# cvg/LightGlue

Hardware: AMD Instinct MI355X
Metric: image-pairs/s at N=M=1024, 9 layers; match-index parity vs ref (higher is better)
Workload: dtype f16; 1 GPU; SuperPoint-dim 256-d descriptors, N=M=1024, 9 layers, pruning/early-stop OFF, batch=32 pairs per GPU, seeded random weights (recipe A), precision=f16x3 (split-f16 operands, 3 MFMAs per product, for every contraction incl. q k^T and P V; fp32 accumulate / residual / softmax); pairs_per_gpu=32, keypoints=1024, keypoints1=1024, descriptor_dim=256, parallelism=pair-sharded dp1, batches_in_flight=1

## Files before the change

### include/lightglue_amd.h

```cpp
#ifndef LIGHTGLUE_AMD_H
#define LIGHTGLUE_AMD_H

#include <stdint.h>

#ifdef __cplusplus
extern "C" {
#endif

enum {
    LG_PREC_F32 = 0,
    LG_PREC_BF16 = 1,
    LG_PREC_F16 = 2,
    LG_PREC_F16X3 = 4
};

#define LG_OK 0
#define LG_ERR_INVALID 1
#define LG_ERR_HIP 2
#define LG_ERR_STATE 3
#define LG_ERR_RANGE 4
#define LG_ERR_DEVICE 5
#define LG_ERR_INDEX 6

#define LG_WIRE_WIDTH(n0, n1) (3LL * (n0) + 3LL * (n1) + 2)
#define LG_MAX_KEYPOINTS 8192
#define LG_MAX_ROWS 2097152
#define LG_MAX_SIM_ELEMS 2147483647LL

typedef struct lg_config {
    int32_t input_dim;
    int32_t descriptor_dim;
    int32_t n_layers;
    int32_t num_heads;
    int32_t add_scale_ori;
    double depth_confidence;
    double width_confidence;
    double filter_threshold;
    int32_t pruning_min_kpts;
    int32_t precision;
    int32_t attn_precision;
} lg_config;

typedef struct lg_engine lg_engine;

#define LG_FLAG_NO_PRUNING 1u
#define LG_FLAG_EXT 2u
#define LG_FLAG_CHECK_FINITE 4u

#define LG_FLAG_INDEXED 8u

typedef struct lg_forward_io {
    int32_t batch, n0, n1;
    uint32_t flags;
    const float *kpts0, *kpts1;
    const float *desc0, *desc1;
    const float *size0, *size1;
    const float *scales0, *oris0, *scales1, *oris1;
    int32_t *matches0, *matches1;
    float *scores0, *scores1;
    int32_t *stop;
    int32_t *prune0, *prune1;
    int32_t *matches;
    float *match_scores;
    int32_t *n_matches;
    const int32_t *num0, *num1;
    float *log_assignment;
    int64_t *matches0_i64, *matches1_i64;
    int64_t *matches_i64;
    int64_t *stop_i64;
    int64_t *prune0_i64, *prune1_i64;
    float *prune0_f32, *prune1_f32;
    int32_t *wire; int64_t wire_stride;
    int32_t *status;
    const int32_t *index0, *index1;
    int32_t images0, images1;
} lg_forward_io;

const char* lg_last_error(void);
const char* lg_version(void);

int lg_engine_create(const lg_config* cfg, lg_engine** out);
void lg_engine_destroy(lg_engine* e);

int lg_engine_set_weight(lg_engine* e, const char* name, const float* host_data, const int64_t* shape, int32_t ndim);
int lg_engine_finalize_weights(lg_engine* e);

int lg_engine_reserve(lg_engine* e, int32_t max_batch, int32_t max_n0, int32_t max_n1);

int lg_engine_forward(lg_engine* e, const lg_forward_io* io, void* hip_stream);

typedef struct lg_unpack_io {
    const int32_t *wire; int64_t wire_stride; int32_t rows;
    int32_t n0, n1, with_prune, pairs_out;
    const int32_t *order;
    int64_t *matches0, *matches1, *stop;
    float *scores0, *scores1;
    int64_t *prune0_i64, *prune1_i64; float *prune0_f32, *prune1_f32;
    int64_t *matches; float *match_scores;
    int32_t *info;
} lg_unpack_io;
int lg_unpack_wire(const lg_unpack_io* io, void* hip_stream);

int lg_engine_set_option(lg_engine* e, const char* key, int32_t value);

int lg_debug_mfma_sustained(double* tflops, double* mhz, void* hip_stream);
int lg_engine_debug_stop_after(lg_engine* e, int32_t step);
int lg_engine_debug_read(lg_engine* e, const char* name, void* host_dst, int64_t max_bytes, int64_t* nbytes_out);
int lg_engine_debug_caps(lg_engine* e, int32_t* cap0, int32_t* cap1);

int32_t lg_profile_num_classes(void);
const char* lg_profile_class_name(int32_t cls);
int lg_engine_profile_enable(lg_engine* e, int32_t on);
int lg_engine_profile_read(lg_engine* e, double* ms, int64_t* count, int32_t n_classes);

int lg_sp_sample_descriptors(const float* desc_map, int32_t batch, int32_t channels, int32_t h, int32_t w,
                             const float* keypoints, const int32_t* num, int32_t n, int32_t cell,
                             int32_t normalize_dense, float* workspace, float* out, void* hip_stream);

int lg_sp_pack_conv_weight(const float* src, int32_t cout, int32_t cin, int32_t k, float* dst, void* hip_stream);
int64_t lg_sp_encode_workspace_bytes(int32_t batch, int32_t h, int32_t w);
int lg_sp_encode(const float* image, int32_t batch, int32_t h, int32_t w, const float* const* params, void* workspace,
                 int64_t workspace_bytes, float* scores, float* desc_map, void* hip_stream);
int lg_sp_pack_conv_weight_split(const float* src, int32_t cout, int32_t cin, int32_t k, void* dst, void* hip_stream);
int lg_sp_encode_split(const float* image, int32_t batch, int32_t h, int32_t w, const float* const* params, void* workspace,
                       int64_t workspace_bytes, float* scores, float* desc_map, void* hip_stream);

int64_t lg_sp_detect_workspace_bytes(int32_t batch, int32_t h, int32_t w, int32_t max_candidates);
int lg_sp_detect(const float* scores, int32_t batch, int32_t h, int32_t w, int32_t nms_radius, int32_t remove_borders,
                 float detection_threshold, int32_t max_keypoints, int32_t capacity, int32_t max_candidates,
                 void* workspace, int64_t workspace_bytes, float* keypoints, float* kp_scores, int32_t* counts,
                 int32_t* totals, void* hip_stream);

int64_t lg_aliked_packed_bytes(int32_t n_pos);
int lg_aliked_pack_weights(int32_t n_pos, const float* const* tensors, int32_t n_tensors, void* packed, int64_t packed_bytes, void* hip_stream);
int64_t lg_aliked_levels_bytes(int32_t batch, int32_t h, int32_t w);
int64_t lg_aliked_workspace_bytes(int32_t batch, int32_t h, int32_t w, int32_t n_pos);
int lg_aliked_encode(const float* image, int32_t batch, int32_t channels, int32_t h, int32_t w, int32_t n_pos, const void* packed, void* levels,
                     void* workspace, int64_t workspace_bytes, float* scores, void* hip_stream);
int64_t lg_aliked_detect_workspace_bytes(int32_t batch, int32_t h, int32_t w, int32_t capacity);
int lg_aliked_detect(const float* scores, int32_t batch, int32_t h, int32_t w, const float* image_size, int32_t nms_radius, float scores_th,
                     int32_t top_k, int32_t n_limit, int32_t capacity, void* workspace, int64_t workspace_bytes, float* keypoints,
                     float* kp_scores, float* kp_norm, int32_t* counts, void* hip_stream);
int64_t lg_aliked_describe_workspace_bytes(int32_t rows, int32_t n_pos);
int lg_aliked_describe(const void* levels, int32_t batch, int32_t h, int32_t w, int32_t n_pos, const void* packed, const float* kp_norm,
                       const int32_t* counts, int32_t n, void* workspace, int64_t workspace_bytes, float* descriptors, void* hip_stream);

#define LG_PREPROCESS_MAX_TAPS 33
#define LG_PREPROCESS_MAX_SIDE 8388608
#define LG_RESIZE_EDGE (-1)
enum { LG_SIDE_LONG = 0, LG_SIDE_SHORT = 1, LG_SIDE_VERT = 2, LG_SIDE_HORZ = 3 };
enum { LG_DTYPE_F32 = 0, LG_DTYPE_U8 = 1 };
typedef struct lg_resize_plan {
    int32_t h_in, w_in, h_out, w_out;
    int32_t ks_y, ks_x;
    int32_t align_corners;
    int32_t identity;
    double sigma_y, sigma_x;
    double scale_x, scale_y;
} lg_resize_plan;
int lg_preprocess_plan(int32_t h, int32_t w, int32_t resize_h, int32_t resize_w, int32_t side, int32_t antialias, int32_t align_corners,
                       lg_resize_plan* plan);
int lg_preprocess_resize(const void* src, int32_t dtype, int32_t batch, int32_t channels, int32_t h, int32_t w, int64_t stride_b,
                         int64_t stride_c, int64_t stride_y, int64_t stride_x, const lg_resize_plan* plan, float* dst, void* hip_stream);

#ifdef __cplusplus
}
#endif
#endif
```

### lightglue_amd/_cabi.py

```python
from __future__ import annotations

import ctypes as C
import os
from pathlib import Path

_LIB_PATH = Path(os.environ.get("LIGHTGLUE_AMD_LIB") or Path(__file__).resolve().parent / "liblightglue_amd.so")

LG_PREC = {"fp32": 0, "bf16": 1, "fp16": 2, "f16x3": 4}
LG_OK, LG_ERR_INVALID, LG_ERR_HIP, LG_ERR_STATE, LG_ERR_RANGE, LG_ERR_DEVICE, LG_ERR_INDEX = 0, 1, 2, 3, 4, 5, 6
LG_FLAG_NO_PRUNING, LG_FLAG_EXT, LG_FLAG_CHECK_FINITE, LG_FLAG_INDEXED = 1, 2, 4, 8
LG_MAX_KEYPOINTS, LG_MAX_ROWS, LG_MAX_SIM_ELEMS = 8192, 2 ** 21, 2 ** 31 - 1

EXPORTED_SYMBOLS = (
    "lg_last_error", "lg_version", "lg_engine_create", "lg_engine_destroy", "lg_engine_set_weight",
    "lg_engine_finalize_weights", "lg_engine_reserve", "lg_engine_forward", "lg_unpack_wire", "lg_engine_set_option",
    "lg_engine_debug_stop_after", "lg_engine_debug_read", "lg_engine_debug_caps",
    "lg_profile_num_classes", "lg_profile_class_name", "lg_engine_profile_enable", "lg_engine_profile_read",
    "lg_sp_sample_descriptors", "lg_sp_detect_workspace_bytes", "lg_sp_detect",
    "lg_sp_pack_conv_weight", "lg_sp_encode_workspace_bytes", "lg_sp_encode", "lg_sp_pack_conv_weight_split", "lg_sp_encode_split", "lg_debug_mfma_sustained",
    "lg_aliked_packed_bytes", "lg_aliked_pack_weights", "lg_aliked_levels_bytes", "lg_aliked_workspace_bytes", "lg_aliked_encode",
    "lg_aliked_detect_workspace_bytes", "lg_aliked_detect", "lg_aliked_describe_workspace_bytes", "lg_aliked_describe",
    "lg_preprocess_plan", "lg_preprocess_resize",
)


class LgConfig(C.Structure):
    _fields_ = [
        ("input_dim", C.c_int32), ("descriptor_dim", C.c_int32), ("n_layers", C.c_int32), ("num_heads", C.c_int32),
        ("add_scale_ori", C.c_int32),
        ("depth_confidence", C.c_double), ("width_confidence", C.c_double), ("filter_threshold", C.c_double),
        ("pruning_min_kpts", C.c_int32), ("precision", C.c_int32), ("attn_precision", C.c_int32),
    ]


_fp = C.c_void_p


class LgForwardIO(C.Structure):
    _fields_ = [
        ("batch", C.c_int32), ("n0", C.c_int32), ("n1", C.c_int32), ("flags", C.c_uint32),
        ("kpts0", _fp), ("kpts1", _fp), ("desc0", _fp), ("desc1", _fp), ("size0", _fp), ("size1", _fp),
        ("scales0", _fp), ("oris0", _fp), ("scales1", _fp), ("oris1", _fp),
        ("matches0", _fp), ("matches1", _fp), ("scores0", _fp), ("scores1", _fp), ("stop", _fp),
        ("prune0", _fp), ("prune1", _fp), ("matches", _fp), ("match_scores", _fp), ("n_matches", _fp),
        ("num0", _fp), ("num1", _fp), ("log_assignment", _fp),
        ("matches0_i64", _fp), ("matches1_i64", _fp), ("matches_i64", _fp), ("stop_i64", _fp),
        ("prune0_i64", _fp), ("prune1_i64", _fp), ("prune0_f32", _fp), ("prune1_f32", _fp),
        ("wire", _fp), ("wire_stride", C.c_int64), ("status", _fp),
        ("index0", _fp), ("index1", _fp), ("images0", C.c_int32), ("images1", C.c_int32),
    ]


class LgUnpackIO(C.Structure):
    _fields_ = [
        ("wire", _fp), ("wire_stride", C.c_int64), ("rows", C.c_int32),
        ("n0", C.c_int32), ("n1", C.c_int32), ("with_prune", C.c_int32), ("pairs_out", C.c_int32),
        ("order", _fp),
        ("matches0", _fp), ("matches1", _fp), ("stop", _fp),
        ("scores0", _fp), ("scores1", _fp),
        ("prune0_i64", _fp), ("prune1_i64", _fp), ("prune0_f32", _fp), ("prune1_f32", _fp),
        ("matches", _fp), ("match_scores", _fp),
        ("info", _fp),
    ]


LG_PREPROCESS_MAX_TAPS, LG_PREPROCESS_MAX_SIDE, LG_RESIZE_EDGE = 33, 2 ** 23, -1
LG_SIDE = {"long": 0, "short": 1, "vert": 2, "horz": 3}
LG_DTYPE_F32, LG_DTYPE_U8 = 0, 1


class LgResizePlan(C.Structure):
    _fields_ = [
        ("h_in", C.c_int32), ("w_in", C.c_int32), ("h_out", C.c_int32), ("w_out", C.c_int32),
        ("ks_y", C.c_int32), ("ks_x", C.c_int32), ("align_corners", C.c_int32), ("identity", C.c_int32),
        ("sigma_y", C.c_double), ("sigma_x", C.c_double), ("scale_x", C.c_double), ("scale_y", C.c_double),
    ]


def wire_width(n0: int, n1: int) -> int:
    return 3 * n0 + 3 * n1 + 2


class LightGlueAmdError(RuntimeError):
    pass


_lib = None


def library_path() -> Path:
    return _LIB_PATH


def load() -> C.CDLL:
    global _lib
    if _lib is not None:
        return _lib
    if not _LIB_PATH.exists():
        raise LightGlueAmdError(
            f"{_LIB_PATH} is missing: build it with `python -c 'import __graft_entry__ as g; g.build()'` "
            f"or `make -C {_LIB_PATH.parent / 'csrc'}`; lightglue_amd has no CPU / PyTorch fallback.")
    lib = C.CDLL(os.fspath(_LIB_PATH))
    lib.lg_last_error.restype = C.c_char_p
    lib.lg_version.restype = C.c_char_p
    lib.lg_engine_create.argtypes = [C.POINTER(LgConfig), C.POINTER(C.c_void_p)]
    lib.lg_engine_destroy.argtypes = [C.c_void_p]
    lib.lg_engine_destroy.restype = None
    lib.lg_engine_set_weight.argtypes = [C.c_void_p, C.c_char_p, C.c_void_p, C.POINTER(C.c_int64), C.c_int32]
    lib.lg_engine_finalize_weights.argtypes = [C.c_void_p]
    lib.lg_engine_reserve.argtypes = [C.c_void_p, C.c_int32, C.c_int32, C.c_int32]
    lib.lg_engine_forward.argtypes = [C.c_void_p, C.POINTER(LgForwardIO), C.c_void_p]
    lib.lg_unpack_wire.argtypes = [C.POINTER(LgUnpackIO), C.c_void_p]
    lib.lg_engine_set_option.argtypes = [C.c_void_p, C.c_char_p, C.c_int32]
    lib.lg_engine_debug_stop_after.argtypes = [C.c_void_p, C.c_int32]
    lib.lg_engine_debug_read.argtypes = [C.c_void_p, C.c_char_p, C.c_void_p, C.c_int64, C.POINTER(C.c_int64)]
    lib.lg_engine_debug_caps.argtypes = [C.c_void_p, C.POINTER(C.c_int32), C.POINTER(C.c_int32)]
    lib.lg_profile_num_classes.restype = C.c_int32
    lib.lg_profile_class_name.restype = C.c_char_p
    lib.lg_profile_class_name.argtypes = [C.c_int32]
    lib.lg_engine_profile_enable.argtypes = [C.c_void_p, C.c_int32]
    lib.lg_engine_profile_read.argtypes = [C.c_void_p, C.POINTER(C.c_double), C.POINTER(C.c_int64), C.c_int32]
    lib.lg_sp_sample_descriptors.argtypes = [C.c_void_p, C.c_int32, C.c_int32, C.c_int32, C.c_int32, C.c_void_p, C.c_void_p,
                                             C.c_int32, C.c_int32, C.c_int32, C.c_void_p, C.c_void_p, C.c_void_p]
    lib.lg_sp_detect_workspace_bytes.argtypes = [C.c_int32] * 4
    lib.lg_sp_detect_workspace_bytes.restype = C.c_int64
    lib.lg_sp_detect.argtypes = [C.c_void_p] + [C.c_int32] * 5 + [C.c_float] + [C.c_int32] * 3 + [C.c_void_p, C.c_int64] + [C.c_void_p] * 5
    lib.lg_sp_pack_conv_weight.argtypes = [C.c_void_p, C.c_int32, C.c_int32, C.c_int32, C.c_void_p, C.c_void_p]
    lib.lg_sp_encode_workspace_bytes.argtypes = [C.c_int32] * 3
    lib.lg_sp_encode_workspace_bytes.restype = C.c_int64
    lib.lg_sp_encode.argtypes = [C.c_void_p, C.c_int32, C.c_int32, C.c_int32, C.POINTER(C.c_void_p), C.c_void_p, C.c_int64, C.c_void_p, C.c_void_p, C.c_void_p]
    lib.lg_sp_pack_conv_weight_split.argtypes = lib.lg_sp_pack_conv_weight.argtypes
    lib.lg_sp_encode_split.argtypes = lib.lg_sp_encode.argtypes
    lib.lg_aliked_packed_bytes.argtypes = [C.c_int32]
    lib.lg_aliked_packed_bytes.restype = C.c_int64
    lib.lg_aliked_pack_weights.argtypes = [C.c_int32, C.POINTER(C.c_void_p), C.c_int32, C.c_void_p, C.c_int64, C.c_void_p]
    lib.lg_aliked_levels_bytes.argtypes = [C.c_int32] * 3
    lib.lg_aliked_levels_bytes.restype = C.c_int64
    lib.lg_aliked_workspace_bytes.argtypes = [C.c_int32] * 4
    lib.lg_aliked_workspace_bytes.restype = C.c_int64
    lib.lg_aliked_encode.argtypes = [C.c_void_p] + [C.c_int32] * 5 + [C.c_void_p] * 3 + [C.c_int64, C.c_void_p, C.c_void_p]
    lib.lg_aliked_detect_workspace_bytes.argtypes = [C.c_int32] * 4
    lib.lg_aliked_detect_workspace_bytes.restype = C.c_int64
    lib.lg_aliked_detect.argtypes = ([C.c_void_p] + [C.c_int32] * 3 + [C.c_void_p, C.c_int32, C.c_float] + [C.c_int32] * 3
                                     + [C.c_void_p, C.c_int64] + [C.c_void_p] * 5)
    lib.lg_aliked_describe_workspace_bytes.argtypes = [C.c_int32] * 2
    lib.lg_aliked_describe_workspace_bytes.restype = C.c_int64
    lib.lg_aliked_describe.argtypes = [C.c_void_p] + [C.c_int32] * 4 + [C.c_void_p] * 3 + [C.c_int32, C.c_void_p, C.c_int64, C.c_void_p, C.c_void_p]
    lib.lg_preprocess_plan.argtypes = [C.c_int32] * 7 + [C.POINTER(LgResizePlan)]
    lib.lg_preprocess_resize.argtypes = [C.c_void_p] + [C.c_int32] * 5 + [C.c_int64] * 4 + [C.POINTER(LgResizePlan), C.c_void_p, C.c_void_p]
    lib.lg_debug_mfma_sustained.argtypes = [C.POINTER(C.c_double), C.POINTER(C.c_double), C.c_void_p]
    _lib = lib
    return lib


def check(rc: int) -> None:
    if rc == LG_OK:
        return
    msg = load().lg_last_error().decode()
    if rc == LG_ERR_INVALID:
        raise AssertionError(msg)
    raise LightGlueAmdError(f"lightglue_amd error {rc}: {msg}")
```

### lightglue_amd/csrc/lg_attention.hip

```cpp
#include "lg_kernels.h"

namespace lg {

constexpr int ABK = 64, ATHREADS = 256;

#ifdef LG_ATTN_TIMING
struct PhaseClock { long long tacc[7] = {0, 0, 0, 0, 0, 0, 0}, tprev = clock64(); };
#define ATT_TICK(pc, slot) do { const long long _n = clock64(); (pc).tacc[slot] += _n - (pc).tprev; (pc).tprev = _n; } while (0)
#else
struct PhaseClock {};
#define ATT_TICK(pc, slot) do { } while (0)
#endif
#ifdef LG_ATTN_WALL
struct WallClock { long long wall0 = wall_clock64(), cyc0 = clock64(); };
#else
struct WallClock {};
#endif
template <int NW> __device__ __forceinline__ long long* dbg_words(const AttnArgs& a) {
    return a.dbg && (threadIdx.x & 63) == 0 ? a.dbg + ((long long)blockIdx.x * NW + (threadIdx.x >> 6)) * 8 : nullptr;
}
template <int NW> __device__ __forceinline__ void dump_timing(const AttnArgs& a, const PhaseClock& pc, int ntiles) {
#ifdef LG_ATTN_TIMING
    if (long long* d = dbg_words<NW>(a)) {
        for (int i = 0; i < 6; ++i) d[i] = pc.tacc[i];
        d[6] = ntiles; d[7] = 1;
    }
#endif
}
template <int NW> __device__ __forceinline__ void dump_wall(const AttnArgs& a, const WallClock& wc, int ntiles) {
#ifdef LG_ATTN_WALL
    if (long long* d = dbg_words<NW>(a)) {
        d[0] = wc.wall0; d[1] = wall_clock64(); d[2] = clock64() - wc.cyc0; d[3] = __builtin_amdgcn_s_getreg((31 << 11) | 4); d[4] = __builtin_amdgcn_s_getreg((31 << 11) | 20); d[6] = ntiles; d[7] = 1;
    }
#endif
}

static int attention_tiles(const RowSpace& rs, int rows) {
    return rows <= 128 ? rs.B * (rs.cap0 + rs.cap1) / rows : rs.B * ((rs.cap0 + rows - 1) / rows + (rs.cap1 + rows - 1) / rows);
}
struct AttnWg { int head; TileLoc t; int qlen, kvseg, kvlen; long long kvbase; };
template <int ABM> __device__ __forceinline__ bool attn_workgroup(const AttnArgs& a, AttnWg& w) {
    const int ntile = gridDim.x >> 2;
    const int v = xcd_remap(blockIdx.x, gridDim.x);
    w.head = v / ntile;
    TileLoc& t = w.t;
    if constexpr (ABM <= 128) {
        t = locate_tile(a.rs, v - w.head * ntile, ABM);
    } else {
        const int t0 = (a.rs.cap0 + ABM - 1) / ABM, t1 = (a.rs.cap1 + ABM - 1) / ABM, idx = v - w.head * ntile;
        t.pair = idx / (t0 + t1);
        const int rem = idx - t.pair * (t0 + t1);
        t.image = rem >= t0 ? 1 : 0;
        t.r0 = (rem - t.image * t0) * ABM;
        t.seg = 2 * t.pair + t.image;
        t.grow0 = seg_row_base(a.rs, t.seg) + t.r0;
    }
    w.qlen = a.rs.len[t.seg];
    if (t.r0 >= w.qlen) return false;
    if (a.rs.active && !a.rs.active[t.pair]) return false;
    w.kvseg = a.cross ? (t.seg ^ 1) : t.seg;
    w.kvlen = a.rs.len[w.kvseg];
    w.kvbase = seg_row_base(a.rs, w.kvseg);
    return true;
}
template <int ABM, int NT> __device__ __forceinline__ void zero_ctx_tile(float* ctx, const AttnWg& w, int tid) {
    for (int i = tid; i < ABM * 16; i += NT) {
        const int row = i >> 4, c4 = i & 15;
        if (w.t.r0 + row < w.qlen) *reinterpret_cast<f32x4*>(ctx + (w.t.grow0 + row) * 256LL + w.head * 64 + c4 * 4) = f32x4{0.f, 0.f, 0.f, 0.f};
    }
}
template <int EPC> __device__ __forceinline__ constexpr int key_of(int kt, int g, int r) {
    return EPC == 8 ? 32 * (kt >> 1) + 8 * g + 4 * (kt & 1) + r : 16 * kt + 4 * g + r;
}
template <int EPC, int QT> __device__ __forceinline__ void mask_dead_keys(f32x4 (&s)[4][QT], const int& g, const int& kv0, const int& kvlen) {
    if (kv0 + ABK > kvlen) {
#pragma unroll
        for (int qt = 0; qt < QT; ++qt)
#pragma unroll
            for (int kt = 0; kt < 4; ++kt)
#pragma unroll
                for (int r = 0; r < 4; ++r)
                    if (kv0 + key_of<EPC>(kt, g, 0) + r >= kvlen) s[kt][qt][r] = -INFINITY;
    }
}
template <int QT> __device__ __forceinline__ float row_max16(const f32x4 (&s)[4][QT], int qt) {
    const float t0 = vmax3(s[0][qt][0], s[0][qt][1], s[0][qt][2]), t1 = vmax3(s[0][qt][3], s[1][qt][0], s[1][qt][1]);
    const float t2 = vmax3(s[1][qt][2], s[1][qt][3], s[2][qt][0]), t3 = vmax3(s[2][qt][1], s[2][qt][2], s[2][qt][3]);
    const float t4 = vmax3(s[3][qt][0], s[3][qt][1], s[3][qt][2]);
    const float mx = vmax2(vmax3(t0, t1, t2), vmax3(t3, t4, s[3][qt][3]));
    return xor32_max(xor16_max(mx));
}
template <bool SUB_M, int QT> __device__ __forceinline__ void exp_sum(f32x4 (&s)[4][QT], const float (&m_run)[QT], float (&l_run)[QT]) {
#pragma unroll
    for (int qt = 0; qt < QT; ++qt) {
        const float nm = m_run[qt];
        auto ex = [&](float x) { if constexpr (SUB_M) return __builtin_amdgcn_exp2f(x - nm); else return __builtin_amdgcn_exp2f(x); };
        float rs0 = 0.f, rs1 = 0.f;
#pragma unroll
        for (int kt = 0; kt < 4; ++kt) {
            const float p0 = ex(s[kt][qt][0]), p1 = ex(s[kt][qt][1]);
            const float p2 = ex(s[kt][qt][2]), p3 = ex(s[kt][qt][3]);
            s[kt][qt][0] = p0; s[kt][qt][1] = p1; s[kt][qt][2] = p2; s[kt][qt][3] = p3;
            rs0 += p0 + p2; rs1 += p1 + p3;
        }
        l_run[qt] += rs0 + rs1;
    }
}
template <int QT> __device__ __forceinline__ void start_rebased(f32x4 (&o)[4][QT], float (&m_run)[QT], float (&l_run)[QT]) {
#pragma unroll
    for (int qt = 0; qt < QT; ++qt) {
        m_run[qt] = 0.f; l_run[qt] = 0.f;
#pragma unroll
        for (int i = 0; i < 4; ++i) o[i][qt] = f32x4{0.f, 0.f, 0.f, 0.f};
    }
}
template <int QT> __device__ __forceinline__ void softmax_rebase(f32x4 (&s)[4][QT], f32x4 (&o)[4][QT], float (&m_run)[QT], float (&l_run)[QT],
                                                                 bool first, int g, int kv0, int kvlen) {
    mask_dead_keys<8>(s, g, kv0, kvlen);
    float dmax[QT];
    bool grew = first;
#pragma unroll
    for (int qt = 0; qt < QT; ++qt) {
        dmax[qt] = row_max16(s, qt);
        grew = grew || (dmax[qt] > 8.f);
    }
    if (__any(grew)) {
#pragma unroll
        for (int qt = 0; qt < QT; ++qt) {
            const float shift = first ? dmax[qt] : (dmax[qt] > 8.f ? dmax[qt] : 0.f);
            const float alpha = first ? 0.f : __builtin_amdgcn_exp2f(-shift);
            l_run[qt] *= alpha;
#pragma unroll
            for (int dt = 0; dt < 4; ++dt) o[dt][qt] *= alpha;
            m_run[qt] += shift;
#pragma unroll
            for (int kt = 0; kt < 4; ++kt) s[kt][qt] -= shift;
        }
    }
}
template <int QT> __device__ __forceinline__ void store_ctx(float* ctx, const TileLoc& t, int head, int qlen, int wave, int lr, int g,
                                                            const f32x4 (&o)[4][QT], const float (&l_run)[QT]) {
#pragma unroll
    for (int qt = 0; qt < QT; ++qt) {
        float l = l_run[qt];
        l = xor32_sum(xor16_sum(l));
        const float inv = 1.f / l;
        const int qrow = t.r0 + wave * (16 * QT) + qt * 16 + lr;
        if (qrow < qlen) {
            float* dst = ctx + (t.grow0 + wave * (16 * QT) + qt * 16 + lr) * 256LL + head * 64 + g * 4;
#pragma unroll
            for (int dt = 0; dt < 4; ++dt) *reinterpret_cast<f32x4*>(dst + dt * 16) = o[dt][qt] * inv;
        }
    }
}
template <class Tag> __device__ __forceinline__ u32x4 mask_tail(u32x4 v, int nvalid) {
    constexpr int EPC = Tag::EPC;
    if (nvalid >= EPC) return v;
    if (nvalid <= 0) return u32x4{0u, 0u, 0u, 0u};
    if constexpr (EPC == 4) {
#pragma unroll
        for (int i = 0; i < 4; ++i) if (i >= nvalid) v[i] = 0u;
    } else {
#pragma unroll
        for (int i = 0; i < 4; ++i) {
            if (2 * i >= nvalid) v[i] = 0u;
            else if (2 * i + 1 >= nvalid) v[i] &= 0xFFFFu;
        }
    }
    return v;
}
__device__ __forceinline__ int k_swz128(int row) { return ((row >> 1) & 1) | (((row >> 3) & 3) << 1); }
template <int ROWB> __device__ __forceinline__ int k_off(int row, int slot16) {
    if constexpr (ROWB == 128) return row * 128 + ((slot16 ^ k_swz128(row)) << 4);
    else return lds_off<ROWB>(row, slot16);
}
template <int PPW, class T> __device__ __forceinline__ void dma_lanes(int wave, int lane, const T* Vt, int head, long long R, long long kvbase,
                                                                      int (&koff)[PPW], const T* (&vrow)[PPW]) {
    const int prow = lane >> 3, pslot = lane & 7;
    int voff[PPW];
#pragma unroll
    for (int i = 0; i < PPW; ++i) {
        const int row = (PPW * wave + i) * 8 + prow;
        koff[i] = row * 64 + ((pslot ^ k_swz128(row)) << 3);
        voff[i] = (pslot ^ lds_swz128(row)) << 3;
    }
#pragma unroll
    for (int i = 0; i < PPW; ++i) vrow[i] = Vt + ((long long)head * 64 + (PPW * wave + i) * 8 + prow) * R + kvbase + voff[i];
}
__device__ __forceinline__ void frag_bases(int lr, int g, int vt, int (&kfo)[2], int (&vfo)[2]) {
#pragma unroll
    for (int c = 0; c < 2; ++c) {
        kfo[c] = k_off<128>(key_of<8>(0, lr >> 2, lr & 3), c * 4 + g);
        vfo[c] = vt + lds_off<128>(lr, 4 * c + g);
    }
}
__device__ __forceinline__ void set_priority_by_progress(int tile, int ntiles) {
    if ((tile & 3) == 0) {
        const int q = (tile * 4) / ntiles;
        if (q == 0) __builtin_amdgcn_s_setprio(3); else if (q == 1) __builtin_amdgcn_s_setprio(2); else if (q == 2) __builtin_amdgcn_s_setprio(1); else __builtin_amdgcn_s_setprio(0);
    }
}
__device__ __forceinline__ void publish_tile() {
    wait_vmcnt0();
    asm volatile("" ::: "memory");
    __syncthreads();
}

template <class Tag, int QT>
__global__ __launch_bounds__(ATHREADS) void attn_kernel(AttnArgs a) {
    constexpr int ABM = 64 * QT;
    typedef typename Tag::elem T;
    constexpr int EPC = Tag::EPC;
    constexpr int ROWB = 64 * (int)sizeof(T);
    constexpr int SLOTS = ROWB / 16;
    constexpr int NC = 64 / (4 * EPC);
    constexpr int NCT = 64 * SLOTS / ATHREADS;
    extern __shared__ __attribute__((aligned(16))) char smem[];
    char* bK = smem;
    char* bV = smem + 64 * ROWB;

    AttnWg w;
    if (!attn_workgroup<ABM>(a, w)) return;
    const int head = w.head, kvlen = w.kvlen;
    const long long kvbase = w.kvbase;
    const int tid = threadIdx.x, lane = tid & 63, wave = tid >> 6, lr = lane & 15, g = lane >> 4;
    const long long R = a.R;
    const T* Q = static_cast<const T*>(a.q);
    const T* Kp = static_cast<const T*>(a.cross ? a.q : a.k);
    const T* Vt = static_cast<const T*>(a.vt);

    if (kvlen == 0) { zero_ctx_tile<ABM, ATHREADS>(a.ctx, w, tid); return; }

    u32x4 qf[QT][NC];
#pragma unroll
    for (int qt = 0; qt < QT; ++qt) {
        const long long grow = min((long long)w.t.grow0 + wave * (16 * QT) + qt * 16 + lr, R - 1);
#pragma unroll
        for (int c = 0; c < NC; ++c)
            qf[qt][c] = *reinterpret_cast<const u32x4*>(Q + ((long long)head * R + grow) * 64 + c * 4 * EPC + g * EPC);
    }

    f32x4 o[4][QT];
    float m_run[QT], l_run[QT];
#pragma unroll
    for (int qt = 0; qt < QT; ++qt) {
        m_run[qt] = -INFINITY; l_run[qt] = 0.f;
#pragma unroll
        for (int i = 0; i < 4; ++i) o[i][qt] = f32x4{0.f, 0.f, 0.f, 0.f};
    }

    u32x4 rk[NCT], rv[NCT];
    auto load_tile = [&](int kv0) {
#pragma unroll
        for (int i = 0; i < NCT; ++i) {
            const int c = tid + ATHREADS * i, row = c / SLOTS, slot = c % SLOTS;
            rk[i] = *reinterpret_cast<const u32x4*>(Kp + ((long long)head * R + kvbase + kv0 + row) * 64 + slot * EPC);
            rv[i] = *reinterpret_cast<const u32x4*>(Vt + ((long long)head * 64 + row) * R + kvbase + kv0 + slot * EPC);
        }
    };
    auto store_tile = [&](int kv0) {
        if (kv0 + ABK <= kvlen) {
#pragma unroll
            for (int i = 0; i < NCT; ++i) {
                const int c = tid + ATHREADS * i, row = c / SLOTS, slot = c % SLOTS;
                *reinterpret_cast<u32x4*>(bK + k_off<ROWB>(row, slot)) = rk[i];
                *reinterpret_cast<u32x4*>(bV + lds_off<ROWB>(row, slot)) = rv[i];
            }
        } else {
#pragma unroll
            for (int i = 0; i < NCT; ++i) {
                const int c = tid + ATHREADS * i, row = c / SLOTS, slot = c % SLOTS;
                const u32x4 kz = (kv0 + row < kvlen) ? rk[i] : u32x4{0u, 0u, 0u, 0u};
                *reinterpret_cast<u32x4*>(bK + k_off<ROWB>(row, slot)) = kz;
                *reinterpret_cast<u32x4*>(bV + lds_off<ROWB>(row, slot)) = mask_tail<Tag>(rv[i], kvlen - (kv0 + slot * EPC));
            }
        }
    };

    const int ntiles = (kvlen + ABK - 1) / ABK;
    PhaseClock pc;
    auto qk = [&](f32x4 (&s)[4][QT]) {
#pragma unroll
        for (int kt = 0; kt < 4; ++kt)
#pragma unroll
            for (int qt = 0; qt < QT; ++qt) s[kt][qt] = f32x4{0.f, 0.f, 0.f, 0.f};
#pragma unroll
        for (int c = 0; c < NC; ++c) {
#pragma unroll
            for (int kt = 0; kt < 4; ++kt) {
                const u32x4 kf = *reinterpret_cast<const u32x4*>(bK + k_off<ROWB>(key_of<EPC>(kt, lr >> 2, lr & 3), c * 4 + g));
#pragma unroll
                for (int qt = 0; qt < QT; ++qt) mma_chunk<Tag>(s[kt][qt], kf, qf[qt][c]);
            }
        }
    };
    auto smax_rescale = [&](f32x4 (&s)[4][QT], int kv0) {
        mask_dead_keys<EPC>(s, g, kv0, kvlen);
        float m_new[QT];
        bool grew = false;
#pragma unroll
        for (int qt = 0; qt < QT; ++qt) {
            m_new[qt] = vmax2(m_run[qt], row_max16(s, qt));
            grew = grew || (m_new[qt] > m_run[qt] + 8.f);
        }
        if (__any(grew)) {
#pragma unroll
            for (int qt = 0; qt < QT; ++qt) {
                const float m_upd = m_new[qt] > m_run[qt] + 8.f ? m_new[qt] : m_run[qt];
                const float alpha = __builtin_amdgcn_exp2f(m_run[qt] - m_upd);
                l_run[qt] *= alpha;
#pragma unroll
                for (int dt = 0; dt < 4; ++dt) o[dt][qt] *= alpha;
                m_run[qt] = m_upd;
            }
        }
    };
    auto pv = [&](f32x4 (&s)[4][QT]) {
        if constexpr (EPC == 8) {
#pragma unroll
            for (int tp = 0; tp < 2; ++tp) {
                u32x4 pp[QT];
#pragma unroll
                for (int qt = 0; qt < QT; ++qt) pp[qt] = pack8<Tag>(s[2 * tp][qt], s[2 * tp + 1][qt]);
#pragma unroll
                for (int dt = 0; dt < 4; ++dt) {
                    const u32x4 vf = *reinterpret_cast<const u32x4*>(bV + lds_off<ROWB>(dt * 16 + lr, 4 * tp + g));
#pragma unroll
                    for (int qt = 0; qt < QT; ++qt) mma_chunk<Tag>(o[dt][qt], vf, pp[qt]);
                }
            }
        } else {
#pragma unroll
            for (int kt = 0; kt < 4; ++kt) {
#pragma unroll
                for (int dt = 0; dt < 4; ++dt) {
                    const u32x4 vf = *reinterpret_cast<const u32x4*>(bV + lds_off<ROWB>(dt * 16 + lr, 4 * kt + g));
#pragma unroll
                    for (int qt = 0; qt < QT; ++qt) mma_chunk<Tag>(o[dt][qt], vf, __builtin_bit_cast(u32x4, s[kt][qt]));
                }
            }
        }
    };

    load_tile(0);
    f32x4 s[4][QT];
    for (int tile = 0; tile < ntiles; ++tile) {
        const int kv0 = tile * ABK;
        __syncthreads();
        ATT_TICK(pc, 0);
        store_tile(kv0);
        __syncthreads();
        ATT_TICK(pc, 1);
        load_tile(tile + 1 < ntiles ? kv0 + ABK : kv0);
        __builtin_amdgcn_sched_barrier(0);
        qk(s);
        ATT_TICK(pc, 2);
        smax_rescale(s, kv0);
        exp_sum<true>(s, m_run, l_run);
        ATT_TICK(pc, 4);
        pv(s);
        ATT_TICK(pc, 5);
    }
    dump_timing<4>(a, pc, ntiles);
    store_ctx(a.ctx, w.t, head, w.qlen, wave, lr, g, o, l_run);
}

template <class Tag>
__global__ __launch_bounds__(ATHREADS, 4) void attn_dma_kernel(AttnArgs a) {
    constexpr int QT = 2, ABM = 128, ROWB = 128, TILEB = 64 * ROWB, BUFB = 2 * TILEB;
    typedef typename Tag::elem T;
    extern __shared__ __attribute__((aligned(16))) char smem[];

    AttnWg w;
    if (!attn_workgroup<ABM>(a, w)) return;
    const int head = w.head, kvlen = w.kvlen;
    const long long kvbase = w.kvbase;
    const int tid = threadIdx.x, lane = tid & 63, wave = __builtin_amdgcn_readfirstlane(tid >> 6), lr = lane & 15, g = lane >> 4;
    const long long R = a.R;
    const T* Q = static_cast<const T*>(a.q);
    const T* Kp = static_cast<const T*>(a.cross ? a.q : a.k);
    const T* Vt = static_cast<const T*>(a.vt);

    if (kvlen == 0) { zero_ctx_tile<ABM, ATHREADS>(a.ctx, w, tid); return; }

    int koff[2];
    const T* vrow[2];
    dma_lanes<2>(wave, lane, Vt, head, R, kvbase, koff, vrow);
    const T* kseg = Kp + ((long long)head * R + kvbase) * 64;
    auto dma_tile = [&](int buf, int kv0) {
        char* bK = smem + buf * BUFB; char* bV = bK + TILEB;
#pragma unroll
        for (int i = 0; i < 2; ++i) {
            lds_dma16(kseg + (long long)kv0 * 64 + koff[i], bK + (2 * wave + i) * 1024);
            lds_dma16(vrow[i] + kv0, bV + (2 * wave + i) * 1024);
        }
    };
    dma_tile(0, 0);

    int kfo[2], vfo[2];
    frag_bases(lr, g, TILEB, kfo, vfo);
    u32x4 qf[QT][2];
#pragma unroll
    for (int qt = 0; qt < QT; ++qt) {
        const long long grow = (long long)w.t.grow0 + wave * 32 + qt * 16 + lr;
#pragma unroll
        for (int c = 0; c < 2; ++c) qf[qt][c] = *reinterpret_cast<const u32x4*>(Q + ((long long)head * R + grow) * 64 + c * 32 + g * 8);
    }
    f32x4 o[4][QT];
    float m_run[QT], l_run[QT];
    start_rebased(o, m_run, l_run);

    const int ntiles = (kvlen + ABK - 1) / ABK;
    PhaseClock pc;
    WallClock wc;
    for (int tile = 0; tile < ntiles; ++tile) {
        const int kv0 = tile * ABK;
        const char* bK = smem + (tile & 1) * BUFB; const char* bV = bK + TILEB;
        set_priority_by_progress(tile, ntiles);
        publish_tile();
        ATT_TICK(pc, 0);
        if (kv0 + ABK > kvlen) {
#pragma unroll
            for (int i = 0; i < 2; ++i) {
                const int c = tid + ATHREADS * i, row = c >> 3, slot = c & 7;
                u32x4* p = reinterpret_cast<u32x4*>(const_cast<char*>(bV) + lds_off<ROWB>(row, slot));
                *p = mask_tail<Tag>(*p, kvlen - (kv0 + slot * 8));
            }
            __syncthreads();
        }
        dma_tile((tile + 1) & 1, tile + 1 < ntiles ? kv0 + ABK : kv0);
        __builtin_amdgcn_sched_barrier(0);
        ATT_TICK(pc, 1);

        f32x4 s[4][QT];
#pragma unroll
        for (int kt = 0; kt < 4; ++kt)
#pragma unroll
            for (int qt = 0; qt < QT; ++qt) s[kt][qt] = f32x4{-m_run[qt], -m_run[qt], -m_run[qt], -m_run[qt]};
#pragma unroll
        for (int c = 0; c < 2; ++c) {
#pragma unroll
            for (int kt = 0; kt < 4; ++kt) {
                const u32x4 kf = *reinterpret_cast<const u32x4*>(bK + kfo[c] + key_of<8>(kt, 0, 0) * ROWB);
#pragma unroll
                for (int qt = 0; qt < QT; ++qt) mma_chunk<Tag>(s[kt][qt], kf, qf[qt][c]);
            }
        }
        ATT_TICK(pc, 2);
        softmax_rebase(s, o, m_run, l_run, tile == 0, g, kv0, kvlen);
        ATT_TICK(pc, 3);
        exp_sum<false>(s, m_run, l_run);
        ATT_TICK(pc, 4);
#pragma unroll
        for (int tp = 0; tp < 2; ++tp) {
            u32x4 pp[QT];
#pragma unroll
            for (int qt = 0; qt < QT; ++qt) pp[qt] = pack8<Tag>(s[2 * tp][qt], s[2 * tp + 1][qt]);
#pragma unroll
            for (int dt = 0; dt < 4; ++dt) {
                const u32x4 vf = *reinterpret_cast<const u32x4*>(bK + vfo[tp] + dt * 16 * ROWB);
#pragma unroll
                for (int qt = 0; qt < QT; ++qt) mma_chunk<Tag>(o[dt][qt], vf, pp[qt]);
            }
        }
        ATT_TICK(pc, 5);
    }
    asm volatile("s_waitcnt vmcnt(0)" ::: "memory");
    dump_timing<4>(a, pc, ntiles);
    dump_wall<4>(a, wc, ntiles);
    store_ctx(a.ctx, w.t, head, w.qlen, wave, lr, g, o, l_run);
}

template <int QT> __device__ __forceinline__ void mma_pair(f32x4 (&acc)[4][QT], int first, const u32x4 (&a)[2], const u32x4 (&b)[QT][2], int c) {
#pragma unroll
    for (int j = 0; j < 2; ++j)
#pragma unroll
        for (int qt = 0; qt < QT; ++qt) mma_chunk<TagF16>(acc[first + j][qt], a[j], b[qt][c]);
}
template <int QT, int NW>
__global__ __launch_bounds__(NW * 64, NW / 2) void attn_split_kernel(AttnArgs a) {
    typedef TagF16 Tag;
    typedef f16_t T;
    constexpr int NT = NW * 64, PPW = 8 / NW;
    constexpr int ABM = 16 * QT * NW, ROWB = 128, TILEB = 64 * ROWB, BUFB = 4 * TILEB;
    extern __shared__ __attribute__((aligned(16))) char smem[];

    AttnWg w;
    if (!attn_workgroup<ABM>(a, w)) return;
    const int head = w.head, kvlen = w.kvlen;
    const long long kvbase = w.kvbase;
    const int tid = threadIdx.x, lane = tid & 63, wave = __builtin_amdgcn_readfirstlane(tid >> 6), lr = lane & 15, g = lane >> 4;
    const long long R = a.R, PL = a.plane;
    const T* Q = static_cast<const T*>(a.q);
    const T* Kp = static_cast<const T*>(a.cross ? a.q : a.k);
    const T* Vt = static_cast<const T*>(a.vt);

    if (kvlen == 0) { zero_ctx_tile<ABM, NT>(a.ctx, w, tid); return; }

    int koff[PPW];
    const T* vrow[PPW];
    dma_lanes<PPW>(wave, lane, Vt, head, R, kvbase, koff, vrow);
    const T* kseg = Kp + ((long long)head * R + kvbase) * 64;
    auto dma_tile = [&](int buf, int kv0) {
        char* bK = smem + buf * BUFB;
#pragma unroll
        for (int i = 0; i < PPW; ++i) {
            const T* ks = kseg + (long long)kv0 * 64 + koff[i];
            const T* vs = vrow[i] + kv0;
            char* dst = bK + (PPW * wave + i) * 1024;
            lds_dma16(ks, dst); lds_dma16(ks + PL, dst + TILEB);
            lds_dma16(vs, dst + 2 * TILEB); lds_dma16(vs + PL, dst + 3 * TILEB);
        }
    };
    dma_tile(0, 0);

    int kfo[2], vfo[2];
    frag_bases(lr, g, 2 * TILEB, kfo, vfo);
    u32x4 qh[QT][2], ql[QT][2];
#pragma unroll
    for (int qt = 0; qt < QT; ++qt) {
        const long long grow = (long long)w.t.grow0 + wave * (16 * QT) + qt * 16 + lr;
#pragma unroll
        for (int c = 0; c < 2; ++c) {
            const T* src = Q + ((long long)head * R + grow) * 64 + c * 32 + g * 8;
            qh[qt][c] = *reinterpret_cast<const u32x4*>(src);
            ql[qt][c] = *reinterpret_cast<const u32x4*>(src + PL);
        }
    }
    f32x4 o[4][QT];
    float m_run[QT], l_run[QT];
    start_rebased(o, m_run, l_run);

    const int ntiles = (kvlen + ABK - 1) / ABK;
    PhaseClock pc;
    WallClock wc;
    for (int tile = 0; tile < ntiles; ++tile) {
        const int kv0 = tile * ABK;
        const char* bK = smem + (tile & 1) * BUFB;
        set_priority_by_progress(tile, ntiles);
        publish_tile();
        ATT_TICK(pc, 0);
        if (kv0 + ABK > kvlen) {
#pragma unroll
            for (int i = 0; i < 1024 / NT; ++i) {
                const int c = (tid + NT * i) & 511, plane = (tid + NT * i) >> 9, row = c >> 3, slot = c & 7;
                u32x4* p = reinterpret_cast<u32x4*>(const_cast<char*>(bK) + (2 + plane) * TILEB + lds_off<ROWB>(row, slot));
                *p = mask_tail<Tag>(*p, kvlen - (kv0 + slot * 8));
            }
            __syncthreads();
        }
        u32x4 fh[2][2], fl[2][2];
        auto load_k = [&](int grp, u32x4 (&h)[2], u32x4 (&l)[2]) {
            const int c = grp >> 1, kp = grp & 1;
#pragma unroll
            for (int j = 0; j < 2; ++j) {
                const char* src = bK + kfo[c] + key_of<8>(2 * kp + j, 0, 0) * ROWB;
                h[j] = *reinterpret_cast<const u32x4*>(src);
                l[j] = *reinterpret_cast<const u32x4*>(src + TILEB);
            }
        };
        auto load_v = [&](int grp, u32x4 (&h)[2], u32x4 (&l)[2]) {
            const int tp = grp >> 1, dp = grp & 1;
#pragma unroll
            for (int j = 0; j < 2; ++j) {
                const char* src = bK + vfo[tp] + (2 * dp + j) * 16 * ROWB;
                h[j] = *reinterpret_cast<const u32x4*>(src);
                l[j] = *reinterpret_cast<const u32x4*>(src + TILEB);
            }
        };
        load_k(0, fh[0], fl[0]);
        dma_tile((tile + 1) & 1, tile + 1 < ntiles ? kv0 + ABK : kv0);
        __builtin_amdgcn_sched_barrier(0);
        ATT_TICK(pc, 1);

        f32x4 s[4][QT];
#pragma unroll
        for (int kt = 0; kt < 4; ++kt)
#pragma unroll
            for (int qt = 0; qt < QT; ++qt) s[kt][qt] = f32x4{-m_run[qt], -m_run[qt], -m_run[qt], -m_run[qt]};
#pragma unroll
        for (int grp = 0; grp < 4; ++grp) {
            const int c = grp >> 1, kp = grp & 1;
            if (grp < 3) load_k(grp + 1, fh[(grp + 1) & 1], fl[(grp + 1) & 1]);
            else load_v(0, fh[0], fl[0]);
            __builtin_amdgcn_sched_barrier(0);
            const u32x4 (&kh)[2] = fh[grp & 1];
            const u32x4 (&kl)[2] = fl[grp & 1];
            mma_pair(s, 2 * kp, kh, ql, c);
            mma_pair(s, 2 * kp, kl, qh, c);
            mma_pair(s, 2 * kp, kh, qh, c);
            __builtin_amdgcn_sched_barrier(0);
        }
        ATT_TICK(pc, 2);
        softmax_rebase(s, o, m_run, l_run, tile == 0, g, kv0, kvlen);
        ATT_TICK(pc, 3);
        exp_sum<false>(s, m_run, l_run);
        ATT_TICK(pc, 4);
        u32x4 ph[QT][2], pl[QT][2];
#pragma unroll
        for (int tp = 0; tp < 2; ++tp)
#pragma unroll
            for (int qt = 0; qt < QT; ++qt) split8_f16<true>(s[2 * tp][qt], s[2 * tp + 1][qt], ph[qt][tp], pl[qt][tp]);
#pragma unroll
        for (int grp = 0; grp < 4; ++grp) {
            const int tp = grp >> 1, dp = grp & 1;
            if (grp < 3) load_v(grp + 1, fh[(grp + 1) & 1], fl[(grp + 1) & 1]);
            __builtin_amdgcn_sched_barrier(0);
            const u32x4 (&vh)[2] = fh[grp & 1];
            const u32x4 (&vl)[2] = fl[grp & 1];
            mma_pair(o, 2 * dp, vh, pl, tp);
            mma_pair(o, 2 * dp, vl, ph, tp);
            mma_pair(o, 2 * dp, vh, ph, tp);
            __builtin_amdgcn_sched_barrier(0);
        }
        ATT_TICK(pc, 5);
    }
    asm volatile("s_waitcnt vmcnt(0)" ::: "memory");
    dump_timing<NW>(a, pc, ntiles);
    dump_wall<NW>(a, wc, ntiles);
    store_ctx(a.ctx, w.t, head, w.qlen, wave, lr, g, o, l_run);
}

template <int QT, int NW> static hipError_t launch_attn_split(const AttnArgs& a, hipStream_t s) {
    if (a.plane <= 0) return hipErrorInvalidValue;
    constexpr int smem = 2 * 4 * 64 * 128;
    auto kern = attn_split_kernel<QT, NW>;
    hipError_t e = hipFuncSetAttribute(reinterpret_cast<const void*>(kern), hipFuncAttributeMaxDynamicSharedMemorySize, smem);
    if (e != hipSuccess) return e;
    hipLaunchKernelGGL(kern, dim3(attention_tiles(a.rs, 16 * QT * NW) * 4), dim3(NW * 64), smem, s, a);
    return hipGetLastError();
}

template <class Tag> static hipError_t launch_attn_dma(const AttnArgs& a, hipStream_t s) {
    hipLaunchKernelGGL((attn_dma_kernel<Tag>), dim3(attention_tiles(a.rs, 128) * 4), dim3(ATHREADS), 2 * 2 * 64 * 128, s, a);
    return hipGetLastError();
}

template <class Tag, int QT> static hipError_t launch_attn_t(const AttnArgs& a, hipStream_t s) {
    constexpr int smem = 2 * 64 * 64 * (int)sizeof(typename Tag::elem);
    hipLaunchKernelGGL((attn_kernel<Tag, QT>), dim3(attention_tiles(a.rs, 64 * QT) * 4), dim3(ATHREADS), smem, s, a);
    return hipGetLastError();
}

template <class Tag> static hipError_t launch_attn_16bit(const AttnArgs& a, hipStream_t s) {
    const int rpw = a.rows_per_wave;
    if (a.dma && rpw == 32) return launch_attn_dma<Tag>(a, s);
    return rpw == 64 ? launch_attn_t<Tag, 4>(a, s) : rpw == 16 ? launch_attn_t<Tag, 1>(a, s) : launch_attn_t<Tag, 2>(a, s);
}

hipError_t launch_attention(int attn_prec, const AttnArgs& a, hipStream_t s) {
    switch (attn_prec) {
        case PREC_F32: return launch_attn_t<TagF32, 2>(a, s);
        case PREC_BF16: return launch_attn_16bit<TagBF16>(a, s);
        case PREC_F16: return launch_attn_16bit<TagF16>(a, s);
        case PREC_F16X3: return a.rows_per_wave == 16 ? launch_attn_split<1, 4>(a, s) : launch_attn_split<1, 8>(a, s);
    }
    return hipErrorInvalidValue;
}

}
```

### lightglue_amd/csrc/lg_common.h

```cpp
#pragma once
#include <hip/hip_runtime.h>
#include <stdint.h>

#if defined(__HIP_DEVICE_COMPILE__) && !defined(__gfx950__)
#error "lightglue_amd kernels are gfx950 (MI355X, CDNA4) only: build with --offload-arch=gfx950"
#endif

namespace lg {

typedef __bf16 bf16_t;
typedef _Float16 f16_t;
typedef float f32x4 __attribute__((ext_vector_type(4)));
typedef float f32x2 __attribute__((ext_vector_type(2)));
typedef __bf16 bf16x8 __attribute__((ext_vector_type(8)));
typedef __bf16 bf16x4 __attribute__((ext_vector_type(4)));
typedef _Float16 f16x8 __attribute__((ext_vector_type(8)));
typedef _Float16 f16x4 __attribute__((ext_vector_type(4)));
typedef uint32_t u32x4 __attribute__((ext_vector_type(4)));
typedef uint32_t u32x2 __attribute__((ext_vector_type(2)));

enum : int { PREC_F32 = 0, PREC_BF16 = 1, PREC_F16 = 2, PREC_F16X3 = 4 };
__host__ __device__ constexpr bool prec_is_split(int prec) { return prec == PREC_F16X3; }

struct TagF32 { typedef float elem; static constexpr int EPC = 4; };
struct TagBF16 { typedef bf16_t elem; static constexpr int EPC = 8; };
struct TagF16 { typedef f16_t elem; static constexpr int EPC = 8; };

template <class Tag> __device__ __forceinline__ void mma_chunk(f32x4& acc, const u32x4& a, const u32x4& b);
template <> __device__ __forceinline__ void mma_chunk<TagBF16>(f32x4& acc, const u32x4& a, const u32x4& b) {
    acc = __builtin_amdgcn_mfma_f32_16x16x32_bf16(__builtin_bit_cast(bf16x8, a), __builtin_bit_cast(bf16x8, b), acc, 0, 0, 0);
}
template <> __device__ __forceinline__ void mma_chunk<TagF16>(f32x4& acc, const u32x4& a, const u32x4& b) {
    acc = __builtin_amdgcn_mfma_f32_16x16x32_f16(__builtin_bit_cast(f16x8, a), __builtin_bit_cast(f16x8, b), acc, 0, 0, 0);
}
template <> __device__ __forceinline__ void mma_chunk<TagF32>(f32x4& acc, const u32x4& a, const u32x4& b) {
    const f32x4 af = __builtin_bit_cast(f32x4, a), bf = __builtin_bit_cast(f32x4, b);
    acc = __builtin_amdgcn_mfma_f32_16x16x4f32(af[0], bf[0], acc, 0, 0, 0);
    acc = __builtin_amdgcn_mfma_f32_16x16x4f32(af[1], bf[1], acc, 0, 0, 0);
    acc = __builtin_amdgcn_mfma_f32_16x16x4f32(af[2], bf[2], acc, 0, 0, 0);
    acc = __builtin_amdgcn_mfma_f32_16x16x4f32(af[3], bf[3], acc, 0, 0, 0);
}

__device__ __forceinline__ uint32_t pack2_bf16(float a, float b) {
    typedef __bf16 bf16x2 __attribute__((ext_vector_type(2)));
    bf16x2 v = {(bf16_t)a, (bf16_t)b};
    return __builtin_bit_cast(uint32_t, v);
}
__device__ __forceinline__ uint32_t pack2_f16(float a, float b) {
    typedef _Float16 f16x2 __attribute__((ext_vector_type(2)));
    f16x2 v = {(f16_t)a, (f16_t)b};
    return __builtin_bit_cast(uint32_t, v);
}
template <class Tag> __device__ __forceinline__ uint32_t pack2(float a, float b);
template <> __device__ __forceinline__ uint32_t pack2<TagBF16>(float a, float b) { return pack2_bf16(a, b); }
template <> __device__ __forceinline__ uint32_t pack2<TagF16>(float a, float b) { return pack2_f16(a, b); }

template <class Tag> __device__ __forceinline__ u32x4 pack8(const f32x4& lo, const f32x4& hi) {
    u32x4 r;
    r[0] = pack2<Tag>(lo[0], lo[1]); r[1] = pack2<Tag>(lo[2], lo[3]);
    r[2] = pack2<Tag>(hi[0], hi[1]); r[3] = pack2<Tag>(hi[2], hi[3]);
    return r;
}
__device__ __forceinline__ void split2_f16(float a, float b, uint32_t& hi, uint32_t& lo) {
    hi = pack2_f16(a, b);
    float la, lb;
    asm("v_fma_mix_f32 %0, %1, -1.0, %2 op_sel_hi:[1,0,0]" : "=v"(la) : "v"(hi), "v"(a));
    asm("v_fma_mix_f32 %0, %1, -1.0, %2 op_sel:[1,0,0] op_sel_hi:[1,0,0]" : "=v"(lb) : "v"(hi), "v"(b));
    lo = pack2_f16(la, lb);
}
template <bool MIX = true>
__device__ __forceinline__ void split8_f16(const f32x4& a, const f32x4& b, u32x4& hi, u32x4& lo) {
    if constexpr (MIX) {
        uint32_t h0, h1, h2, h3, l0, l1, l2, l3;
        split2_f16(a[0], a[1], h0, l0); split2_f16(a[2], a[3], h1, l1);
        split2_f16(b[0], b[1], h2, l2); split2_f16(b[2], b[3], h3, l3);
        hi = u32x4{h0, h1, h2, h3}; lo = u32x4{l0, l1, l2, l3};
    } else {
        float h[8], l[8];
#pragma unroll
        for (int i = 0; i < 4; ++i) { h[i] = (float)(f16_t)a[i]; l[i] = a[i] - h[i]; h[4 + i] = (float)(f16_t)b[i]; l[4 + i] = b[i] - h[4 + i]; }
        hi[0] = pack2_f16(h[0], h[1]); hi[1] = pack2_f16(h[2], h[3]); hi[2] = pack2_f16(h[4], h[5]); hi[3] = pack2_f16(h[6], h[7]);
        lo[0] = pack2_f16(l[0], l[1]); lo[1] = pack2_f16(l[2], l[3]); lo[2] = pack2_f16(l[4], l[5]); lo[3] = pack2_f16(l[6], l[7]);
    }
}
template <class Tag> __device__ __forceinline__ void split8(const f32x4& a, const f32x4& b, u32x4& hi, u32x4& lo);
template <> __device__ __forceinline__ void split8<TagF16>(const f32x4& a, const f32x4& b, u32x4& hi, u32x4& lo) { split8_f16<false>(a, b, hi, lo); }

__device__ __forceinline__ int lds_swz128(int row) { return (row >> 1) & 7; }
template <int ROWB> __device__ __forceinline__ int lds_off(int row, int slot16) {
    if constexpr (ROWB == 128) return row * 128 + ((slot16 ^ lds_swz128(row)) << 4);
    else return row * 256 + ((slot16 ^ (row & 15)) << 4);
}

__device__ __forceinline__ void lds_dma16(const void* gptr, void* lds) {
    const uint32_t dst = __builtin_amdgcn_readfirstlane((uint32_t)(uintptr_t)(__attribute__((address_space(3))) void*)lds);
    asm volatile("s_mov_b32 m0, %0\n\ts_nop 0\n\tglobal_load_lds_dwordx4 %1, off" :: "s"(dst), "v"(gptr) : "memory", "m0");
}

__device__ __forceinline__ void lds_dma16_s(const void* sbase, uint32_t voff, void* lds) {
    const uint32_t dst = __builtin_amdgcn_readfirstlane((uint32_t)(uintptr_t)(__attribute__((address_space(3))) void*)lds);
    const uint64_t b = (uint64_t)(uintptr_t)sbase;
    const uint32_t blo = __builtin_amdgcn_readfirstlane((uint32_t)b), bhi = __builtin_amdgcn_readfirstlane((uint32_t)(b >> 32));
    const uint64_t sb = ((uint64_t)bhi << 32) | blo;
    asm volatile("s_mov_b32 m0, %0\n\ts_nop 0\n\tglobal_load_lds_dwordx4 %1, %2" :: "s"(dst), "v"(voff), "s"(sb) : "memory", "m0");
}

__device__ __forceinline__ void wait_vmcnt0() { __builtin_amdgcn_s_waitcnt(0x0F70); }

__device__ __forceinline__ __amdgpu_buffer_rsrc_t weight_rsrc(const void* base) {
    return __builtin_amdgcn_make_buffer_rsrc(const_cast<void*>(base), 0, 0x7FFFFFF0, 0x00020000);
}
__device__ __forceinline__ u32x4 weight_frag(__amdgpu_buffer_rsrc_t rs, int lane_off, int byte_off) {
    return __builtin_amdgcn_raw_buffer_load_b128(rs, lane_off, byte_off, 0);
}

struct RowSpace {
    int B;
    int cap0, cap1;
    const int* len;
    const int* active;
};
struct TileLoc { int pair, image, seg, r0, grow0; };
__device__ __forceinline__ TileLoc locate_tile(const RowSpace& rs, int tile, int tile_rows) {
    TileLoc t;
    const int per_pair = rs.cap0 + rs.cap1;
    t.grow0 = tile * tile_rows;
    t.pair = t.grow0 / per_pair;
    const int rem = t.grow0 - t.pair * per_pair;
    t.image = rem >= rs.cap0 ? 1 : 0;
    t.r0 = rem - t.image * rs.cap0;
    t.seg = 2 * t.pair + t.image;
    return t;
}
__device__ __forceinline__ int seg_row_base(const RowSpace& rs, int seg) {
    return (seg >> 1) * (rs.cap0 + rs.cap1) + (seg & 1) * rs.cap0;
}

struct PairIndex { const int* index0; const int* index1; int images0, images1; };
__device__ __forceinline__ int source_image(const PairIndex& px, int pair, int image) {
    if (!px.index0) return pair;
    const int s0 = px.index0[pair], s1 = px.index1[pair];
    if ((unsigned)s0 >= (unsigned)px.images0 || (unsigned)s1 >= (unsigned)px.images1) return -1;
    return image ? s1 : s0;
}

__device__ __forceinline__ int rr_rotate(int id, int nwg) {
    if (id >= (nwg & ~7)) return id;
    const int q = id >> 3;
    return (q << 3) + ((id + q) & 7);
}

__device__ __forceinline__ int xcd_remap(int id, int nwg) {
    const int q = nwg >> 3, r = nwg & 7, xcd = id & 7, k = id >> 3;
    return (xcd < r ? xcd * (q + 1) : r * (q + 1) + (xcd - r) * q) + k;
}

template <int CTRL> __device__ __forceinline__ float dpp_mov(float v) {
    return __builtin_bit_cast(float, __builtin_amdgcn_update_dpp(0, __builtin_bit_cast(int, v), CTRL, 0xF, 0xF, true));
}
__device__ __forceinline__ float vmax2(float a, float b) { float r; asm("v_max_f32 %0, %1, %2" : "=v"(r) : "v"(a), "v"(b)); return r; }
__device__ __forceinline__ float vmax3(float a, float b, float c) { float r; asm("v_max3_f32 %0, %1, %2, %3" : "=v"(r) : "v"(a), "v"(b), "v"(c)); return r; }

struct SwapPair { float a, b; };
__device__ __forceinline__ SwapPair swap16(float x) {
    const auto r = __builtin_amdgcn_permlane16_swap(__builtin_bit_cast(unsigned, x), __builtin_bit_cast(unsigned, x), false, false);
    const unsigned lo = r[0], hi = r[1];
    return {__builtin_bit_cast(float, lo), __builtin_bit_cast(float, hi)};
}
__device__ __forceinline__ SwapPair swap32(float x) {
    const auto r = __builtin_amdgcn_permlane32_swap(__builtin_bit_cast(unsigned, x), __builtin_bit_cast(unsigned, x), false, false);
    const unsigned lo = r[0], hi = r[1];
    return {__builtin_bit_cast(float, lo), __builtin_bit_cast(float, hi)};
}
__device__ __forceinline__ float xor16_max(float x) { const SwapPair p = swap16(x); return vmax2(p.a, p.b); }
__device__ __forceinline__ float xor32_max(float x) { const SwapPair p = swap32(x); return vmax2(p.a, p.b); }
__device__ __forceinline__ float xor16_sum(float x) { const SwapPair p = swap16(x); return p.a + p.b; }
__device__ __forceinline__ float xor32_sum(float x) { const SwapPair p = swap32(x); return p.a + p.b; }
__device__ __forceinline__ float dpp_xor1(float v) { return dpp_mov<0xB1>(v); }
__device__ __forceinline__ float dpp_xor2(float v) { return dpp_mov<0x4E>(v); }
__device__ __forceinline__ float row16_sum(float v) {
    v += dpp_xor1(v);
    v += dpp_xor2(v);
    v += dpp_mov<0x141>(v);
    v += dpp_mov<0x140>(v);
    return v;
}

template <class F> __device__ __forceinline__ void wave_allreduce2(float& x0, float& x1, F merge) {
    merge(x0, x1, dpp_xor1(x0), dpp_xor1(x1));
    merge(x0, x1, dpp_xor2(x0), dpp_xor2(x1));
    merge(x0, x1, dpp_mov<0x141>(x0), dpp_mov<0x141>(x1));
    merge(x0, x1, dpp_mov<0x140>(x0), dpp_mov<0x140>(x1));
    { const SwapPair p0 = swap16(x0), p1 = swap16(x1); x0 = p0.a; x1 = p1.a; merge(x0, x1, p0.b, p1.b); }
    { const SwapPair p0 = swap32(x0), p1 = swap32(x1); x0 = p0.a; x1 = p1.a; merge(x0, x1, p0.b, p1.b); }
}

__device__ __forceinline__ float wave_allmax(float x) {
    x = vmax2(x, dpp_xor1(x)); x = vmax2(x, dpp_xor2(x)); x = vmax2(x, dpp_mov<0x141>(x)); x = vmax2(x, dpp_mov<0x140>(x));
    return xor32_max(xor16_max(x));
}
__device__ __forceinline__ float wave_allsum(float x) { return xor32_sum(xor16_sum(row16_sum(x))); }

__device__ __forceinline__ float wave_sum(float v) {
#pragma unroll
    for (int o = 32; o > 0; o >>= 1) v += __shfl_xor(v, o, 64);
    return v;
}
__device__ __forceinline__ float wave_max(float v) {
#pragma unroll
    for (int o = 32; o > 0; o >>= 1) v = fmaxf(v, __shfl_xor(v, o, 64));
    return v;
}

}
```

### lightglue_amd/csrc/lg_debug.hip

```cpp
#include "lg_engine.h"

using namespace lg;

static const char* const kProfNames[LG_PROF_NCLS] = {"prep", "gemm_qkv_self", "attn_self", "gemm_out_proj", "gemm_ffn0", "ln_gelu", "gemm_ffn3_resid",
    "gemm_qkv_cross", "attn_cross", "adaptive", "rowdot", "gemm_final_proj", "sim", "assign", "fused_tail"};

namespace lg {

int prof_begin(lg_engine* e, int cls, hipStream_t s) {
    e->prof_open = e->profiling && (e->prof_only < 0 || e->prof_only == cls);
    if (!e->prof_open) return LG_OK;
    if (e->prof_used == e->prof_pool.size()) {
        lg_engine::ProfSpan sp{};
        HIPCHK(hipEventCreate(&sp.a)); HIPCHK(hipEventCreate(&sp.b));
        e->prof_pool.push_back(sp);
    }
    e->prof_pool[e->prof_used].cls = cls;
    HIPCHK(hipEventRecord(e->prof_pool[e->prof_used].a, s));
    return LG_OK;
}
int prof_end(lg_engine* e, hipStream_t s) {
    if (!e->prof_open) return LG_OK;
    e->prof_open = false;
    HIPCHK(hipEventRecord(e->prof_pool[e->prof_used].b, s));
    e->prof_used++;
    return LG_OK;
}

}

namespace {

int prof_collect(lg_engine* e) {
    for (size_t i = 0; i < e->prof_used; ++i) {
        HIPCHK(hipEventSynchronize(e->prof_pool[i].b));
        float ms = 0.f;
        HIPCHK(hipEventElapsedTime(&ms, e->prof_pool[i].a, e->prof_pool[i].b));
        e->prof_ms[e->prof_pool[i].cls] += ms;
        e->prof_cnt[e->prof_pool[i].cls] += 1;
    }
    e->prof_used = 0;
    return LG_OK;
}

__global__ __launch_bounds__(512) void mfma_spin_kernel(long long* cycles, int iters) {
    typedef __bf16 bf16x8_t __attribute__((ext_vector_type(8)));
    const unsigned h = (threadIdx.x * 2654435761u + blockIdx.x * 40503u) * 12345u;
    u32x4 xa = {h ^ 0x3f803f80u, (h >> 3) | 0x3c003c00u, (h * 7u) & 0x3fff3fffu, (h * 13u) & 0x3fff3fffu};
    u32x4 xb = {(h * 3u) & 0x3fff3fffu, (h * 5u) & 0x3fff3fffu, (h * 11u) & 0x3fff3fffu, (h * 17u) & 0x3fff3fffu};
    f32x4 acc[8];
    for (int i = 0; i < 8; ++i) acc[i] = f32x4{0.f, 0.f, 0.f, 0.f};
    const long long t0 = clock64();
    for (int it = 0; it < iters; ++it) {
        asm volatile("" : "+v"(xa), "+v"(xb));
#pragma unroll
        for (int i = 0; i < 8; ++i) acc[i] = __builtin_amdgcn_mfma_f32_16x16x32_bf16(__builtin_bit_cast(bf16x8_t, xa), __builtin_bit_cast(bf16x8_t, xb), acc[i], 0, 0, 0);
    }
    const long long t1 = clock64();
    float sacc = 0.f;
    for (int i = 0; i < 8; ++i) sacc += acc[i][0];
    if ((threadIdx.x & 63) == 0) atomicMax(reinterpret_cast<unsigned long long*>(cycles), (unsigned long long)(t1 - t0));
    if (sacc == 12345.f) cycles[1] = 1;
}

}

extern "C" {

int32_t lg_profile_num_classes(void) { return LG_PROF_NCLS; }
const char* lg_profile_class_name(int32_t cls) { return (cls >= 0 && cls < LG_PROF_NCLS) ? kProfNames[cls] : ""; }
int lg_engine_profile_enable(lg_engine* e, int32_t on) {
    if (!e) return set_error(LG_ERR_INVALID, "null engine");
    if (!on && e->profiling) { int rc = prof_collect(e); if (rc != LG_OK) return rc; }
    e->profiling = on != 0;
    return LG_OK;
}
int lg_engine_profile_read(lg_engine* e, double* ms, int64_t* count, int32_t n) {
    if (!e || !ms || !count || n < LG_PROF_NCLS) return set_error(LG_ERR_INVALID, "bad argument");
    int rc = prof_collect(e);
    if (rc != LG_OK) return rc;
    for (int i = 0; i < LG_PROF_NCLS; ++i) { ms[i] = e->prof_ms[i]; count[i] = e->prof_cnt[i]; e->prof_ms[i] = 0; e->prof_cnt[i] = 0; }
    return LG_OK;
}

int lg_engine_debug_stop_after(lg_engine* e, int32_t step) { if (!e) return set_error(LG_ERR_INVALID, "null engine"); e->debug_stop = step; return LG_OK; }

int lg_debug_mfma_sustained(double* tflops, double* mhz, void* hip_stream) {
    if (!tflops || !mhz) return set_error(LG_ERR_INVALID, "null pointer");
    hipStream_t s = static_cast<hipStream_t>(hip_stream);
    long long* d = nullptr;
    HIPCHK(hipMalloc(&d, 16));
    hipEvent_t a, b;
    HIPCHK(hipEventCreate(&a)); HIPCHK(hipEventCreate(&b));
    const int iters = 400000;
    hipLaunchKernelGGL(mfma_spin_kernel, dim3(256), dim3(512), 0, s, d, iters / 10);
    HIPCHK(hipMemsetAsync(d, 0, 16, s));
    HIPCHK(hipEventRecord(a, s));
    hipLaunchKernelGGL(mfma_spin_kernel, dim3(256), dim3(512), 0, s, d, iters);
    HIPCHK(hipEventRecord(b, s));
    HIPCHK(hipEventSynchronize(b));
    float ms = 0.f; long long h[2] = {0, 0};
    HIPCHK(hipEventElapsedTime(&ms, a, b));
    HIPCHK(hipMemcpy(h, d, 16, hipMemcpyDeviceToHost));
    (void)hipFree(d); (void)hipEventDestroy(a); (void)hipEventDestroy(b);
    *mhz = ms > 0.f ? (double)h[0] / (ms * 1e3) : 0.0;
    *tflops = ms > 0.f ? 256.0 * 8.0 * iters * 8.0 * 16384.0 / (ms * 1e9) : 0.0;
    return LG_OK;
}

int lg_engine_debug_caps(lg_engine* e, int32_t* cap0, int32_t* cap1) {
    if (!e || !cap0 || !cap1) return set_error(LG_ERR_INVALID, "null argument");
    *cap0 = e->cur_cap0; *cap1 = e->cur_cap1;
    return LG_OK;
}

int lg_engine_debug_read(lg_engine* e, const char* name, void* host_dst, int64_t max_bytes, int64_t* nbytes_out) {
    if (!e || !name) return set_error(LG_ERR_INVALID, "null argument");
    auto it = e->bufs.find(name);
    if (it == e->bufs.end()) return set_error(LG_ERR_INVALID, std::string("unknown buffer '") + name + "'");
    if (nbytes_out) *nbytes_out = (int64_t)it->second.second;
    HIPCHK(hipDeviceSynchronize());
    if (host_dst && max_bytes > 0) {
        const size_t n = (size_t)max_bytes < it->second.second ? (size_t)max_bytes : it->second.second;
        HIPCHK(hipMemcpy(host_dst, it->second.first, n, hipMemcpyDeviceToHost));
    }
    return LG_OK;
}

}
```

### lightglue_amd/csrc/lg_engine.h

```cpp
#pragma once
#include <hip/hip_runtime.h>

#include <cstring>
#include <map>
#include <string>
#include <vector>

#include "../../include/lightglue_amd.h"
#include "lg_kernels.h"

#define TRY(x) do { int _rc = (x); if (_rc != LG_OK) return _rc; } while (0)

enum { PC_PREP = 0, PC_GEMM_QKV_SELF, PC_ATTN_SELF, PC_GEMM_OUT, PC_GEMM_FFN1, PC_LN_GELU, PC_GEMM_FFN2, PC_GEMM_QKV_CROSS,
       PC_ATTN_CROSS, PC_ADAPTIVE, PC_ROWDOT, PC_GEMM_FINAL, PC_SIM, PC_ASSIGN, PC_TAIL, LG_PROF_NCLS };

namespace lg {

struct HostTensor { std::vector<float> data; std::vector<int64_t> shape; };

struct PackedW { void* hi = nullptr; void* lo = nullptr; };

inline size_t elem_size(int prec) { return prec == PREC_F32 ? 4 : 2; }

struct Arena {
    char* base = nullptr; size_t used = 0;
    template <class T> void take(T*& member, size_t bytes) {
        used = (used + 255) & ~size_t(255);
        if (base) member = reinterpret_cast<T*>(base + used);
        used += bytes;
    }
};

struct BlockWeights {
    int Nout, n_qk_groups;
    PackedW out, f1, f2;
    float *b_qkv = nullptr, *b_out = nullptr, *b_f1 = nullptr, *b_f2 = nullptr;
    float *ln_g = nullptr, *ln_b = nullptr;
    char *tail_cat = nullptr, *tail_2 = nullptr;
    float* b_cat = nullptr;
    char* qkv_p = nullptr; size_t qkv_layer_bytes = 0;
};

}

struct lg_engine {
    lg_config cfg{};
    int attn_prec = 0;
    std::map<std::string, lg::HostTensor> staged;
    bool weights_ready = false;
    void* w_arena = nullptr;
    lg::BlockWeights blocks[2] = {{768, 2}, {512, 1}};
    lg::PackedW w_in;
    float *b_in = nullptr, *b_final = nullptr;
    float *w_match = nullptr, *b_match = nullptr, *w_tok = nullptr, *b_tok = nullptr;
    float* Wr = nullptr;
    size_t tail_cat_layer_bytes = 0, tail_2_layer_bytes = 0;
    char* w_final_p = nullptr; size_t final_layer_bytes = 0;
    bool attn_dma = true;
    int attn_rows = 32;
    int fused_tail = 1, fused_next = 1, fused_prep = 1;
    int tail_timing = 0; long long* TAILDBG = nullptr; long long* TAILDBG2 = nullptr;
    int* CFLAGS = nullptr; int compact_epoch = 0; bool cflags_clean = false;
    int tail_row_tiles = 0;
    bool attn_auto_rows = true;
    void* ws = nullptr; size_t ws_bytes = 0;
    int capB = 0, cap0 = 0, cap1 = 0;
    int cur_cap0 = 0, cur_cap1 = 0, curB = 0;
    std::map<std::string, std::pair<void*, size_t>> bufs;
    float *X, *CTX, *MSG, *H1, *G, *COS, *SIN, *MD, *SIM, *LS, *LSNEG, *CONF, *MSCORE, *LSE_R, *LSE_C, *MAX0, *MAX1, *BBOX, *XIN, *CPM, *CPS, *CBV;
    int* CBI;
    void *Q, *K, *VT;
    int *IND, *DST, *LEN, *LEN_ORIG, *LEN_OLD, *ACTIVE, *FINAL_LAYER, *ARG0, *ARG1;
    int* RANGEF = nullptr;
    float *X2 = nullptr, *COS2 = nullptr, *SIN2 = nullptr; int* XSEL = nullptr;
    bool adapt_gather = true;
    bool sim_planes = true;
    int sim_chunk = 0;
    int debug_stop = -1;
    bool profiling = false, prof_open = false;
    int prof_only = -1;
    struct ProfSpan { hipEvent_t a, b; int cls; };
    std::vector<ProfSpan> prof_pool;
    size_t prof_used = 0;
    double prof_ms[LG_PROF_NCLS] = {0};
    long long prof_cnt[LG_PROF_NCLS] = {0};
};

namespace lg {

size_t weight_layout(lg_engine* e, char* base);
size_t workspace_layout(lg_engine* e, char* base, int B, int c0, int c1);

int prof_begin(lg_engine* e, int cls, hipStream_t s);
int prof_end(lg_engine* e, hipStream_t s);

}
```

### lightglue_amd/csrc/lg_engine.hip

```cpp
#include <cmath>
#include <cstring>
#include <string>

#include "lg_engine.h"

using namespace lg;

namespace {

inline int round_up(int x, int m) { return (x + m - 1) / m * m; }
size_t attn_elem_bytes(int attn_prec) { return attn_prec == PREC_F32 ? 4 : attn_prec == PREC_F16X3 ? 4 : 2; }
int compact_chunks(int c0, int c1) { return (c0 > c1 ? c0 : c1) / compact_chunk_rows(); }
size_t cflags_bytes(int B, int c0, int c1) { return (size_t)2 * B * compact_chunks(c0, c1) * 4 + 256; }

}

namespace lg {

size_t workspace_layout(lg_engine* e, char* base, int B, int c0, int c1) {
    const size_t R = (size_t)B * (c0 + c1), as = attn_elem_bytes(e->attn_prec);
    const size_t per0 = (size_t)B * c0 * 4, per1 = (size_t)B * c1 * 4, tiles = (size_t)B * (c0 / 32) * c1 * 4;
    Arena ar{base};
    if (base) e->bufs.clear();
    auto take = [&](const char* name, auto*& member, size_t bytes) { ar.take(member, bytes); if (base) e->bufs[name] = {member, bytes}; };
    take("X", e->X, R * 256 * 4); take("CTX", e->CTX, R * 256 * 4); take("MSG", e->MSG, R * 256 * 4);
    take("H1", e->H1, R * 512 * 4); take("G", e->G, R * 512 * 4);
    take("COS", e->COS, R * 32 * 4); take("SIN", e->SIN, R * 32 * 4);
    take("MD", e->MD, R * 256 * 4);
    take("SIM", e->SIM, (size_t)B * c0 * c1 * 4);
    take("LS", e->LS, R * 4); take("LSNEG", e->LSNEG, R * 4); take("CONF", e->CONF, R * 4); take("MSCORE", e->MSCORE, R * 4);
    take("LSE_R", e->LSE_R, per0); take("LSE_C", e->LSE_C, per1);
    take("MAX0", e->MAX0, per0); take("MAX1", e->MAX1, per1);
    take("ARG0", e->ARG0, per0); take("ARG1", e->ARG1, per1);
    take("CPM", e->CPM, tiles); take("CPS", e->CPS, tiles); take("CBV", e->CBV, tiles); take("CBI", e->CBI, tiles);
    take("BBOX", e->BBOX, (size_t)B * 8 * 4);
    take("XIN", e->XIN, R * (size_t)e->cfg.input_dim * 4);
    take("Q", e->Q, R * 256 * as); take("K", e->K, R * 256 * as); take("VT", e->VT, R * 256 * as);
    take("IND", e->IND, R * 4); take("DST", e->DST, R * 4);
    take("LEN", e->LEN, (size_t)B * 2 * 4); take("LEN_ORIG", e->LEN_ORIG, (size_t)B * 2 * 4); take("LEN_OLD", e->LEN_OLD, (size_t)B * 2 * 4);
    take("ACTIVE", e->ACTIVE, (size_t)B * 4); take("FINAL_LAYER", e->FINAL_LAYER, (size_t)B * 4);
    take("RANGEF", e->RANGEF, (size_t)B * 4);
    take("XSEL", e->XSEL, (size_t)B * 4);
    take("X2", e->X2, R * 256 * 4); take("COS2", e->COS2, R * 32 * 4); take("SIN2", e->SIN2, R * 32 * 4);
    take("CFLAGS", e->CFLAGS, cflags_bytes(B, c0, c1));
    take("TAILDBG", e->TAILDBG, R * 16); take("TAILDBG2", e->TAILDBG2, R * 16);
    return ar.used;
}

}

static int ensure_workspace(lg_engine* e, int B, int n0, int n1) {
    const int c0 = round_up(n0 > 0 ? n0 : 1, 128), c1 = round_up(n1 > 0 ? n1 : 1, 128);
    const bool fits = e->ws && B <= e->capB && c0 <= e->cap0 && c1 <= e->cap1;
    if (!fits) {
        if (e->ws) { HIPCHK(hipDeviceSynchronize()); HIPCHK(hipFree(e->ws)); e->ws = nullptr; }
        e->capB = B > e->capB ? B : e->capB; e->cap0 = c0 > e->cap0 ? c0 : e->cap0; e->cap1 = c1 > e->cap1 ? c1 : e->cap1;
        e->ws_bytes = workspace_layout(e, nullptr, e->capB, e->cap0, e->cap1);
        HIPCHK(hipMalloc(&e->ws, e->ws_bytes));
    }
    if (fits && e->curB == B && e->cur_cap0 == c0 && e->cur_cap1 == c1 && !e->bufs.empty()) return LG_OK;
    e->curB = B; e->cur_cap0 = c0; e->cur_cap1 = c1;
    e->cflags_clean = false;
    if (workspace_layout(e, static_cast<char*>(e->ws), B, c0, c1) > e->ws_bytes) return set_error(LG_ERR_STATE, "workspace carve overflow");
    return LG_OK;
}

extern "C" {

int lg_engine_create(const lg_config* cfg, lg_engine** out) {
    if (!cfg || !out) return set_error(LG_ERR_INVALID, "null argument");
    if (cfg->descriptor_dim != 256 || cfg->num_heads != 4) return set_error(LG_ERR_INVALID, "only descriptor_dim=256, num_heads=4 (head_dim 64) are built");
    if (cfg->n_layers < 1 || cfg->n_layers > 64) return set_error(LG_ERR_INVALID, "bad n_layers");
    if (cfg->input_dim <= 0 || cfg->input_dim % 64) return set_error(LG_ERR_INVALID, "input_dim must be a positive multiple of 64");
    if (cfg->precision != LG_PREC_F32 && cfg->precision != LG_PREC_BF16 && cfg->precision != LG_PREC_F16 && cfg->precision != LG_PREC_F16X3) return set_error(LG_ERR_INVALID, "bad precision");
    auto* e = new lg_engine();
    e->cfg = *cfg;
    int ap = cfg->attn_precision;
    if (ap < 0) ap = cfg->precision;
    if (!(ap == cfg->precision || (cfg->precision == PREC_F16X3 && ap == PREC_F16))) { delete e; return set_error(LG_ERR_INVALID, "bad attn_precision: must equal `precision`, or LG_PREC_F16 with LG_PREC_F16X3"); }
    e->attn_prec = ap;
    *out = e;
    return LG_OK;
}

void lg_engine_destroy(lg_engine* e) {
    if (!e) return;
    for (auto& sp : e->prof_pool) { (void)hipEventDestroy(sp.a); (void)hipEventDestroy(sp.b); }
    if (e->ws) (void)hipFree(e->ws);
    if (e->w_arena) (void)hipFree(e->w_arena);
    delete e;
}

static int check_envelope(long long B, long long n0, long long n1) {
    const long long c0 = (n0 + 127) / 128 * 128, c1 = (n1 + 127) / 128 * 128;
    if (n0 > LG_MAX_KEYPOINTS || n1 > LG_MAX_KEYPOINTS)
        return set_error(LG_ERR_INVALID, "more than LG_MAX_KEYPOINTS (8192) keypoints in one image");
    if (B * (c0 + c1) > LG_MAX_ROWS)
        return set_error(LG_ERR_INVALID, "batch * (cap0 + cap1) exceeds LG_MAX_ROWS (2^21 keypoint rows per forward): split the batch across calls");
    if (B * c0 * c1 > LG_MAX_SIM_ELEMS)
        return set_error(LG_ERR_INVALID, "batch * cap0 * cap1 exceeds LG_MAX_SIM_ELEMS (2^31 - 1 similarity entries per forward): split the batch across calls");
    return LG_OK;
}

int lg_engine_reserve(lg_engine* e, int32_t max_batch, int32_t max_n0, int32_t max_n1) {
    if (!e || max_batch < 1 || max_n0 < 0 || max_n1 < 0) return set_error(LG_ERR_INVALID, "bad argument");
    TRY(check_envelope(max_batch, max_n0, max_n1));
    return ensure_workspace(e, max_batch, max_n0, max_n1);
}

int lg_engine_set_option(lg_engine* e, const char* key, int32_t value) {
    if (!e || !key) return set_error(LG_ERR_INVALID, "null argument");
    if (std::strcmp(key, "fused_tail") == 0) { e->fused_tail = value != 0; return LG_OK; }
    if (std::strcmp(key, "fused_next") == 0) { e->fused_next = value != 0; return LG_OK; }
    if (std::strcmp(key, "fused_prep") == 0) { e->fused_prep = value != 0; return LG_OK; }
    if (std::strcmp(key, "attn_dma") == 0) { e->attn_dma = value != 0; return LG_OK; }
    if (std::strcmp(key, "adapt_gather") == 0) { e->adapt_gather = value != 0; return LG_OK; }
    if (std::strcmp(key, "sim_planes") == 0) { e->sim_planes = value != 0; return LG_OK; }
    if (std::strcmp(key, "sim_chunk") == 0) { if (value < 0 || value % 64) return set_error(LG_ERR_INVALID, "sim_chunk: 0 or a multiple of 64"); e->sim_chunk = value; return LG_OK; }
    if (std::strcmp(key, "attn_rows") == 0) { if (value != 16 && value != 32 && value != 64) return set_error(LG_ERR_INVALID, "attn_rows must be 16, 32 or 64"); e->attn_rows = value; e->attn_auto_rows = false; return LG_OK; }
    if (std::strcmp(key, "tail_row_tiles") == 0) { if (value != 0 && value != 1 && value != 2 && value != 4) return set_error(LG_ERR_INVALID, "tail_row_tiles must be 0 (automatic), 1, 2 or 4"); e->tail_row_tiles = value; return LG_OK; }
    if (std::strcmp(key, "profile_only") == 0) { e->prof_only = value; return LG_OK; }
    if (std::strcmp(key, "tail_timing") == 0) { e->tail_timing = value; return LG_OK; }
    return set_error(LG_ERR_INVALID, std::string("unknown option '") + key + "'");
}

namespace {
int tail_row_tiles_for(int R) {
    int best = 4; long long best_cost = -1;
    const int shapes[3] = {4, 2, 1}; const long long cost[3] = {114, 69, 58};
    for (int i = 0; i < 3; ++i) {
        const long long wgs = R / (16 * shapes[i]), rounds = (wgs + 255) / 256, c = rounds * cost[i];
        if (best_cost < 0 || c < best_cost) { best = shapes[i]; best_cost = c; }
    }
    return best;
}

bool pruning_on(const lg_engine* e, const lg_forward_io* io) { return e->cfg.width_confidence > 0 && !(io->flags & LG_FLAG_NO_PRUNING); }
bool indexed(const lg_forward_io* io) { return (io->flags & LG_FLAG_EXT) && (io->flags & LG_FLAG_INDEXED); }
PairIndex pair_index(const lg_forward_io* io) { return indexed(io) ? PairIndex{io->index0, io->index1, io->images0, io->images1} : PairIndex{}; }

int check_forward_io(const lg_engine* e, const lg_forward_io* io) {
    if (!e || !io) return set_error(LG_ERR_INVALID, "null argument");
    if (!e->weights_ready) return set_error(LG_ERR_STATE, "weights not finalised");
    const int B = io->batch, n0 = io->n0, n1 = io->n1;
    if (B < 1 || n0 < 0 || n1 < 0) return set_error(LG_ERR_INVALID, "bad batch / keypoint counts");
    TRY(check_envelope(B, n0, n1));
    if (!io->stop || !io->n_matches) return set_error(LG_ERR_INVALID, "null output pointer");
    if ((n0 && (!io->matches0 || !io->scores0)) || (n1 && (!io->matches1 || !io->scores1))) return set_error(LG_ERR_INVALID, "null output pointer");
    if (n0 && n1 && (!io->matches || !io->match_scores)) return set_error(LG_ERR_INVALID, "null match-list pointer");
    if (n0 && n1 && (!io->kpts0 || !io->kpts1 || !io->desc0 || !io->desc1)) return set_error(LG_ERR_INVALID, "null input pointer");
    const bool do_prune = pruning_on(e, io);
    if (do_prune && ((n0 && !io->prune0) || (n1 && !io->prune1))) return set_error(LG_ERR_INVALID, "prune0/prune1 required when width_confidence > 0");
    if (e->cfg.add_scale_ori && (!io->scales0 || !io->oris0 || !io->scales1 || !io->oris1)) return set_error(LG_ERR_INVALID, "scales/oris required");
    const bool ext = (io->flags & LG_FLAG_EXT) != 0;
    if ((io->flags & LG_FLAG_CHECK_FINITE) && (!ext || !io->status)) return set_error(LG_ERR_INVALID, "LG_FLAG_CHECK_FINITE needs LG_FLAG_EXT and a status array");
    if (io->flags & LG_FLAG_INDEXED) {
        if (!ext || !io->status) return set_error(LG_ERR_INVALID, "LG_FLAG_INDEXED needs LG_FLAG_EXT and a status array");
        if (!io->index0 || !io->index1) return set_error(LG_ERR_INVALID, "LG_FLAG_INDEXED: null index0 / index1");
        if (io->images0 < 1 || io->images1 < 1) return set_error(LG_ERR_INVALID, "LG_FLAG_INDEXED: images0 and images1 must be at least 1");
    }
    if (ext && io->wire && io->wire_stride < LG_WIRE_WIDTH(n0, n1)) return set_error(LG_ERR_INVALID, "wire_stride < LG_WIRE_WIDTH(n0, n1) = 3 n0 + 3 n1 + 2");
    if (ext && do_prune && ((io->prune0_f32 || io->prune1_f32))) return set_error(LG_ERR_INVALID, "prune0_f32 / prune1_f32 are the outputs of a forward WITHOUT pruning");
    if (ext && !do_prune && ((io->prune0_i64 || io->prune1_i64))) return set_error(LG_ERR_INVALID, "prune0_i64 / prune1_i64 are the outputs of a forward WITH pruning");
    return LG_OK;
}

hipError_t write_outputs(const lg_engine* e, const lg_forward_io* io, const int* final_layer, int stop_const, const int* range_flag, const int* device_err, hipStream_t s) {
    OutArgs o{};
    o.B = io->batch; o.n0 = io->n0; o.n1 = io->n1; o.L = e->cfg.n_layers; o.kmax = io->n0 < io->n1 ? io->n0 : io->n1;
    o.final_layer = final_layer; o.stop_const = stop_const; o.stop = io->stop;
    o.m0 = io->matches0; o.m1 = io->matches1; o.s0 = io->scores0; o.s1 = io->scores1; o.matches = io->matches; o.n_matches = io->n_matches;
    o.prune0 = io->prune0; o.prune1 = io->prune1; o.num0 = io->num0; o.num1 = io->num1;
    if (io->flags & LG_FLAG_EXT) {
        o.m0_64 = (long long*)io->matches0_i64; o.m1_64 = (long long*)io->matches1_i64; o.matches_64 = (long long*)io->matches_i64; o.stop_64 = (long long*)io->stop_i64;
        o.prune0_64 = (long long*)io->prune0_i64; o.prune1_64 = (long long*)io->prune1_i64; o.prune0_f = io->prune0_f32; o.prune1_f = io->prune1_f32;
        o.wire = io->wire; o.wire_stride = io->wire_stride; o.wire_prune = pruning_on(e, io) ? 1 : 0; o.status = io->status; o.range_flag = range_flag; o.device_err = device_err;
        o.px = pair_index(io);
    }
    return launch_write_outputs(o, s);
}

int forward_empty(const lg_engine* e, const lg_forward_io* io, hipStream_t s) {
    const int B = io->batch, n0 = io->n0, n1 = io->n1;
    if (n0) { HIPCHK(hipMemsetAsync(io->matches0, 0xFF, sizeof(int) * (size_t)B * n0, s)); HIPCHK(hipMemsetAsync(io->scores0, 0, 4 * (size_t)B * n0, s)); }
    if (n1) { HIPCHK(hipMemsetAsync(io->matches1, 0xFF, sizeof(int) * (size_t)B * n1, s)); HIPCHK(hipMemsetAsync(io->scores1, 0, 4 * (size_t)B * n1, s)); }
    HIPCHK(hipMemsetAsync(io->n_matches, 0, sizeof(int) * (size_t)B, s));
    InitStateArgs is{};
    is.B = B; is.n0 = n0; is.n1 = n1; is.L = e->cfg.n_layers; is.px = pair_index(io);
    if (pruning_on(e, io)) { is.prune0 = n0 ? io->prune0 : nullptr; is.prune1 = n1 ? io->prune1 : nullptr; }
    HIPCHK(launch_init_state(is, s));
    HIPCHK(write_outputs(e, io, nullptr, 1, nullptr, nullptr, s));
    return LG_OK;
}
}

int lg_engine_forward(lg_engine* e, const lg_forward_io* io, void* hip_stream) {
    TRY(check_forward_io(e, io));
    hipStream_t s = static_cast<hipStream_t>(hip_stream);
    const int B = io->batch, n0 = io->n0, n1 = io->n1, L = e->cfg.n_layers, D = 256;
    if (n0 == 0 || n1 == 0) return forward_empty(e, io, s);
    const bool do_stop = e->cfg.depth_confidence > 0, do_prune = pruning_on(e, io);
    const bool check_finite = (io->flags & LG_FLAG_EXT) && (io->flags & LG_FLAG_CHECK_FINITE);
    const int max_matches = n0 < n1 ? n0 : n1;

    TRY(ensure_workspace(e, B, n0, n1));
    const int c0 = e->cur_cap0, c1 = e->cur_cap1, R = B * (c0 + c1);
    RowSpace rs_all{B, c0, c1, e->LEN, nullptr};
    RowSpace rs_act{B, c0, c1, e->LEN, e->ACTIVE};
    const int prec = e->cfg.precision, ap = e->attn_prec;
    int step = 0;
#define STEP_DONE() do { if (e->debug_stop >= 0 && step >= e->debug_stop) return LG_OK; ++step; } while (0)
#define PROFILED(cls, launch) do { TRY(prof_begin(e, cls, s)); HIPCHK(launch); TRY(prof_end(e, s)); } while (0)

    int* const device_err = e->CFLAGS + (size_t)2 * B * compact_chunks(c0, c1);
    const InitStateArgs is{B, n0, n1, L, io->num0, io->num1, e->LEN, e->LEN_ORIG, e->LEN_OLD, e->ACTIVE, e->FINAL_LAYER,
                           do_prune ? io->prune0 : nullptr, do_prune ? io->prune1 : nullptr, e->RANGEF, device_err, e->XSEL, pair_index(io)};
    HIPCHK(launch_init_state(is, s));
    int* const range_flag = check_finite ? e->RANGEF : nullptr;
    const bool fuse_prep = e->fused_prep && e->cfg.input_dim == D && e->debug_stop < 0 && e->tail_timing != 2;
    PrepArgs p{};
    p.rs = rs_all; p.n0 = n0; p.n1 = n1; p.px = pair_index(io); p.kpts0 = io->kpts0; p.kpts1 = io->kpts1; p.size0 = io->size0; p.size1 = io->size1;
    p.scales0 = io->scales0; p.oris0 = io->oris0; p.scales1 = io->scales1; p.oris1 = io->oris1;
    p.Wr = e->Wr; p.pos_dim = 2 + 2 * (e->cfg.add_scale_ori ? 1 : 0);
    p.desc0 = io->desc0; p.desc1 = io->desc1; p.input_dim = e->cfg.input_dim;
    p.X = e->X; p.Xin = e->XIN; p.cosb = e->COS; p.sinb = e->SIN; p.ind = e->IND; p.bbox = e->BBOX;
    TRY(prof_begin(e, PC_PREP, s));
    if (fuse_prep) HIPCHK(launch_prep_bbox(p, s)); else HIPCHK(launch_prep(p, s));
    auto gemm = [&](const RowSpace& rs, const float* A, int lda, const float* A2, int lda2, int K1, int K, const PackedW& W, size_t w_elems, const float* bias, int Nout, float* out) {
        GemmArgs g{};
        g.rs = rs; g.A = A; g.lda = lda; g.A2 = A2; g.lda2 = lda2; g.K1 = K1; g.K = K; g.bias = bias; g.Nout = Nout; g.out = out; g.ldo = Nout; g.out_scale = 1.f; g.R = R;
        g.W = static_cast<char*>(W.hi) + w_elems * elem_size(prec); g.Wlo = W.lo ? static_cast<char*>(W.lo) + w_elems * elem_size(prec) : nullptr;
        return g;
    };
    if (e->cfg.input_dim != D) {
        GemmArgs g = gemm(rs_all, e->XIN, e->cfg.input_dim, nullptr, 0, e->cfg.input_dim, e->cfg.input_dim, e->w_in, 0, e->b_in, D, e->X);
        HIPCHK(launch_gemm(prec, EPI_STORE, g, s));
    }
    TRY(prof_end(e, s));
    STEP_DONE();
    const long long qkv_plane = ap == PREC_F16X3 ? (long long)R * 256 : 0;

    int xcur = 0;
    float* Xs[2] = {e->X, e->X2}; float* Cs[2] = {e->COS, e->COS2}; float* Ss[2] = {e->SIN, e->SIN2};
    bool gather_pending = false;
    auto make_proj = [&](int layer, int blk) {
        ProjArgs pj{};
        pj.rs = rs_act; pj.X = Xs[xcur]; pj.R = R; pj.q = e->Q; pj.k = e->K; pj.vt = e->VT; pj.plane = qkv_plane;
        const BlockWeights& bw = e->blocks[blk];
        pj.W = bw.qkv_p + (size_t)layer * bw.qkv_layer_bytes; pj.bias = bw.b_qkv + (size_t)layer * bw.Nout;
        pj.Nout = bw.Nout; pj.n_qk_groups = bw.n_qk_groups;
        if (blk == 0) { pj.cosb = Cs[xcur]; pj.sinb = Ss[xcur]; }
        pj.dbg = nullptr; pj.range_flag = range_flag;
        return pj;
    };
    const bool fuse_next = e->fused_next && e->fused_tail && (e->tail_timing == 0 || e->tail_timing == 5 || e->tail_timing == 6) &&
                           e->debug_stop < 0 && launch_tail_supports_next(prec, ap);
    const bool prune_possible = do_prune && (n0 > e->cfg.pruning_min_kpts || n1 > e->cfg.pruning_min_kpts);
    const bool use_gather = e->adapt_gather && e->fused_tail && e->debug_stop < 0 && e->tail_timing == 0;
    bool proj_done = false, final_done = false;
    auto make_final = [&](const RowSpace& rs, int layer, bool per_pair) {
        FinalArgs f{};
        f.rs = rs; f.X = per_pair ? e->X : Xs[xcur]; f.R = R; f.out = e->MD; f.scale = 0.25f;
        f.planes = (prec == PREC_F16X3 && e->sim_planes) ? 1 : 0;
        if (per_pair) { f.X2 = e->X2; f.xsel = e->XSEL; }
        f.W = e->w_final_p + (per_pair ? 0 : (size_t)layer * e->final_layer_bytes); f.bias = e->b_final + (per_pair ? 0 : (size_t)layer * D);
        f.layer_of_pair = per_pair ? e->FINAL_LAYER : nullptr; f.w_layer_bytes = (long long)e->final_layer_bytes;
        return f;
    };
    for (int i = 0; i < L; ++i) {
        for (int blk = 0; blk < 2; ++blk) {
            const BlockWeights& bw = e->blocks[blk];
            if (!proj_done) {
                ProjArgs pj = make_proj(i, blk);
                pj.dbg = (e->tail_timing == 2 && blk == 0) ? e->TAILDBG : nullptr;
                TRY(prof_begin(e, blk == 0 ? PC_GEMM_QKV_SELF : PC_GEMM_QKV_CROSS, s));
                if (fuse_prep && i == 0 && blk == 0) {
                    pj.rs = rs_all;
                    if (launch_proj_first(prec, ap, pj, p, s) != hipSuccess) {
                        (void)hipGetLastError();
                        HIPCHK(launch_prep(p, s));
                        pj.rs = rs_act;
                        HIPCHK(launch_proj(prec, ap, pj, s));
                    }
                }
                else if (gather_pending && blk == 0) {
                    GatherArgs ga{};
                    ga.Xold = Xs[xcur]; ga.cos_old = Cs[xcur]; ga.sin_old = Ss[xcur]; ga.Xnew = Xs[xcur ^ 1]; ga.cos_new = Cs[xcur ^ 1]; ga.sin_new = Ss[xcur ^ 1];
                    ga.src = e->DST; ga.len_old = e->LEN_OLD;
                    HIPCHK(launch_proj_gather(prec, ap, pj, ga, s));
                    xcur ^= 1; gather_pending = false;
                }
                else HIPCHK(launch_proj(prec, ap, pj, s));
                TRY(prof_end(e, s));
            }
            proj_done = false;
            STEP_DONE();
            {
                AttnArgs at{};
                at.rs = rs_act; at.q = e->Q; at.k = e->K; at.vt = e->VT; at.plane = qkv_plane; at.ctx = e->CTX; at.R = R; at.cross = blk;
                at.dbg = (e->tail_timing == 3 && blk == 0) ? e->TAILDBG : nullptr;
                at.rows_per_wave = (e->attn_auto_rows && R / 128 * 4 < 256) ? 16 : e->attn_rows; at.dma = e->attn_dma ? 1 : 0;
                PROFILED(blk == 0 ? PC_ATTN_SELF : PC_ATTN_CROSS, launch_attention(ap, at, s));
            }
            STEP_DONE();
            if (e->fused_tail) {
                TailArgs ta{};
                ta.rs = rs_act; ta.X = Xs[xcur]; ta.CTX = e->CTX; ta.range_flag = range_flag;
                ta.Wcat = bw.tail_cat + (size_t)i * e->tail_cat_layer_bytes; ta.bcat = bw.b_cat + (size_t)i * 512;
                ta.gamma = bw.ln_g + (size_t)i * 512; ta.beta = bw.ln_b + (size_t)i * 512;
                ta.W2 = bw.tail_2 + (size_t)i * e->tail_2_layer_bytes; ta.b2 = bw.b_f2 + (size_t)i * D;
                if (blk == 1) {
                    const bool last = i + 1 == L;
                    const bool prune_here = !last && do_prune && prune_possible;
                    const bool want_tok = !last && do_stop, want_ls = last || do_stop;
                    if (want_tok) { ta.head_w0 = e->w_tok + (size_t)i * D; ta.head_b0 = e->b_tok + i; ta.head_out0 = e->CONF; }
                    if (prune_here || want_ls) {
                        float* sig = prune_here ? e->MSCORE : nullptr; float* ls = want_ls ? e->LS : nullptr;
                        float* lsneg = (want_ls && io->log_assignment) ? e->LSNEG : nullptr;
                        if (want_tok) { ta.head_w1 = e->w_match + (size_t)i * D; ta.head_b1 = e->b_match + i; ta.head_out1 = sig; ta.head_ls1 = ls; ta.head_lsneg1 = lsneg; }
                        else { ta.head_w0 = e->w_match + (size_t)i * D; ta.head_b0 = e->b_match + i; ta.head_out0 = sig; ta.head_ls0 = ls; ta.head_lsneg0 = lsneg; }
                    }
                }
                ta.dbg = (e->tail_timing == 1 || (i == 0 && ((e->tail_timing == 5 && blk == 1) || (e->tail_timing == 6 && blk == 0)))) ? e->TAILDBG : nullptr;
                ta.row_tiles = e->tail_row_tiles ? e->tail_row_tiles : tail_row_tiles_for(R);
                if (fuse_next && (blk == 0 || (i + 1 < L && !prune_possible))) {
                    ta.next = make_proj(i + blk, blk ^ 1);
                    if (ta.dbg && e->tail_timing >= 5) ta.next.dbg = e->TAILDBG2;
                    proj_done = true;
                } else if (fuse_next && blk == 1 && i + 1 == L && !do_stop) {
                    ta.fin = make_final(rs_act, L - 1, false);
                    final_done = true;
                }
                PROFILED(PC_TAIL, launch_tail(prec, ap, ta, s));
                STEP_DONE(); STEP_DONE(); STEP_DONE(); STEP_DONE();
                continue;
            }
            {
                GemmArgs g = gemm(rs_act, e->CTX, D, nullptr, 0, D, D, bw.out, (size_t)i * D * D, bw.b_out + (size_t)i * D, D, e->MSG);
                PROFILED(PC_GEMM_OUT, launch_gemm(prec, EPI_STORE, g, s));
            }
            STEP_DONE();
            {
                GemmArgs g = gemm(rs_act, e->X, D, e->MSG, D, D, 512, bw.f1, (size_t)i * 512 * 512, bw.b_f1 + (size_t)i * 512, 512, e->H1);
                PROFILED(PC_GEMM_FFN1, launch_gemm(prec, EPI_STORE, g, s));
            }
            STEP_DONE();
            {
                LnGeluArgs ln{rs_act, e->H1, e->G, bw.ln_g + (size_t)i * 512, bw.ln_b + (size_t)i * 512, R};
                PROFILED(PC_LN_GELU, launch_ln_gelu(ln, s));
            }
            STEP_DONE();
            {
                GemmArgs g = gemm(rs_act, e->G, 512, nullptr, 0, 512, 512, bw.f2, (size_t)i * D * 512, bw.b_f2 + (size_t)i * D, D, e->X);
                PROFILED(PC_GEMM_FFN2, launch_gemm(prec, EPI_RESID, g, s));
            }
            STEP_DONE();
        }
        if (i == L - 1) break;
        const bool prune_now = do_prune && prune_possible;
        if (do_stop || prune_now) {
            if (!e->fused_tail) {
                RowDotArgs rd{};
                rd.rs = rs_act; rd.X = e->X;
                if (do_stop) { rd.w0 = e->w_tok + (size_t)i * D; rd.b0 = e->b_tok + i; rd.out0 = e->CONF; rd.act0 = 1; }
                if (do_stop && prune_now) { rd.w1 = e->w_match + (size_t)i * D; rd.b1 = e->b_match + i; rd.out1 = e->MSCORE; rd.act1 = 1; }
                else if (prune_now) { rd.w0 = e->w_match + (size_t)i * D; rd.b0 = e->b_match + i; rd.out0 = e->MSCORE; rd.act0 = 1; }
                PROFILED(PC_ROWDOT, launch_rowdot(rd, s));
            }
            AdaptArgs ad{};
            ad.rs = rs_act; ad.len = e->LEN; ad.active = e->ACTIVE; ad.len_old = e->LEN_OLD; ad.final_layer = e->FINAL_LAYER;
            ad.ind = e->IND; ad.dst = e->DST; ad.prune0 = io->prune0; ad.prune1 = io->prune1; ad.n0 = n0; ad.n1 = n1; ad.len_orig = e->LEN_ORIG;
            ad.conf = e->CONF; ad.mscore = e->MSCORE; ad.X = e->X; ad.cosb = e->COS; ad.sinb = e->SIN;
            if (use_gather && prune_now) { ad.gather = 1; ad.src = e->DST; ad.xsel = e->XSEL; ad.xnext = xcur ^ 1; gather_pending = true; }
            ad.layer = i;
            ad.conf_thr = (float)std::fmin(std::fmax(0.8 + 0.1 * std::exp(-4.0 * i / L), 0.0), 1.0);
            ad.depth_conf = (float)e->cfg.depth_confidence;
            ad.width_conf = (float)(1.0 - e->cfg.width_confidence);
            ad.pruning_min_kpts = e->cfg.pruning_min_kpts;
            ad.do_stop = do_stop; ad.do_prune = prune_now;
            ad.compact_chunks = compact_chunks(c0, c1); ad.compact_flags = e->CFLAGS; ad.compact_err = device_err; ad.compact_ticket = device_err + 1;
            if (prune_now && !e->cflags_clean) {
                HIPCHK(hipMemsetAsync(e->CFLAGS, 0, cflags_bytes(B, c0, c1), s));
                e->cflags_clean = true;
            }
            ad.compact_epoch = ++e->compact_epoch;
            PROFILED(PC_ADAPTIVE, launch_adapt(ad, s));
        }
    }
    {
        if (!e->fused_tail) {
            RowDotArgs rd{};
            rd.rs = rs_all; rd.X = e->X; rd.w0 = e->w_match; rd.b0 = e->b_match; rd.out0 = e->LS; rd.act0 = 2;
            rd.layer_of_pair = e->FINAL_LAYER; rd.w_layer_stride = D; rd.ignore_active = 1;
            if (io->log_assignment) { rd.w1 = e->w_match; rd.b1 = e->b_match; rd.out1 = e->LSNEG; rd.act1 = 3; }
            PROFILED(PC_ROWDOT, launch_rowdot(rd, s));
        }
        if (!final_done) {
            PROFILED(PC_GEMM_FINAL, launch_final_proj(prec, make_final(rs_all, 0, true), s));
        }
        TRY(prof_begin(e, PC_SIM, s));
        if (prec == PREC_F16X3 && e->sim_planes) {
            SimPlanesArgs sp{rs_all, reinterpret_cast<const f16_t*>(e->MD), (long long)R * 256, D, e->SIM, e->sim_chunk};
            HIPCHK(launch_sim_planes(sp, s));
        } else {
            SimArgs sm{rs_all, e->MD, D, D, e->SIM};
            HIPCHK(launch_sim(prec, sm, s));
        }
        TRY(prof_end(e, s));
        AssignArgs as{};
        as.rs = rs_all; as.sim = e->SIM; as.ls = e->LS; as.lse_r = e->LSE_R; as.lse_c = e->LSE_C; as.max0 = e->MAX0; as.arg0 = e->ARG0;
        as.max1 = e->MAX1; as.arg1 = e->ARG1; as.cpm = e->CPM; as.cps = e->CPS; as.cbv = e->CBV; as.cbi = e->CBI; as.ind = e->IND; as.n0 = n0; as.n1 = n1; as.filter_threshold = (float)e->cfg.filter_threshold;
        as.m0 = io->matches0; as.m1 = io->matches1; as.s0 = io->scores0; as.s1 = io->scores1;
        as.matches = io->matches; as.mscores = io->match_scores; as.n_matches = io->n_matches; as.max_matches = max_matches;
        as.log_assignment = io->log_assignment; as.lsneg = e->LSNEG;
        as.dbg = e->tail_timing == 4 ? e->TAILDBG : nullptr;
        as.all_rows_live = (!do_prune && !io->num0 && !io->num1 && !indexed(io)) ? 1 : 0;
        PROFILED(PC_ASSIGN, launch_assign(as, s));
        HIPCHK(write_outputs(e, io, e->FINAL_LAYER, 0, range_flag, device_err, s));
    }
#undef PROFILED
#undef STEP_DONE
    return LG_OK;
}

}
```

### lightglue_amd/csrc/lg_pointwise.hip

```cpp
#include "lg_kernels.h"

namespace lg {

__global__ __launch_bounds__(256) void bbox_kernel(PrepArgs a) {
    const int seg = blockIdx.x, image = seg & 1, pair = seg >> 1;
    const int n = image ? a.n1 : a.n0;
    const int live = a.rs.len[seg];
    const float* kp = (image ? a.kpts1 : a.kpts0) + (long long)source_image(a.px, pair, image) * n * 2;
    float mnx = INFINITY, mny = INFINITY, mxx = -INFINITY, mxy = -INFINITY;
    for (int i = threadIdx.x; i < live; i += 256) {
        const float x = kp[2 * i], y = kp[2 * i + 1];
        mnx = fminf(mnx, x); mny = fminf(mny, y); mxx = fmaxf(mxx, x); mxy = fmaxf(mxy, y);
    }
    __shared__ float sh[4][4];
    mnx = -wave_max(-mnx); mny = -wave_max(-mny); mxx = wave_max(mxx); mxy = wave_max(mxy);
    const int w = threadIdx.x >> 6;
    if ((threadIdx.x & 63) == 0) { sh[w][0] = mnx; sh[w][1] = mny; sh[w][2] = mxx; sh[w][3] = mxy; }
    __syncthreads();
    if (threadIdx.x == 0) {
        for (int i = 1; i < 4; ++i) { mnx = fminf(mnx, sh[i][0]); mny = fminf(mny, sh[i][1]); mxx = fmaxf(mxx, sh[i][2]); mxy = fmaxf(mxy, sh[i][3]); }
        float* o = a.bbox + seg * 4;
        o[0] = mnx; o[1] = mny; o[2] = mxx; o[3] = mxy;
    }
}

__global__ __launch_bounds__(256) void prep_kernel(PrepArgs a) {
    const int wave = threadIdx.x >> 6, lane = threadIdx.x & 63;
    const int seg = blockIdx.y, image = seg & 1, pair = seg >> 1;
    const int n = image ? a.n1 : a.n0;
    const int r = blockIdx.x * 4 + wave;
    if (r >= a.rs.len[seg]) return;
    const long long grow = seg_row_base(a.rs, seg) + r;
    const long long src = source_image(a.px, pair, image);
    const float* kp = (image ? a.kpts1 : a.kpts0) + (src * n + r) * 2;
    const float* szp = image ? a.size1 : a.size0;
    float sx, sy;
    if (szp) { sx = szp[src * 2]; sy = szp[src * 2 + 1]; }
    else { const float* bb = a.bbox + seg * 4; sx = 1.f + bb[2] - bb[0]; sy = 1.f + bb[3] - bb[1]; }
    const float scale = fmaxf(sx, sy) / 2.f;
    float kn[4];
    kn[0] = (kp[0] - sx / 2.f) / scale;
    kn[1] = (kp[1] - sy / 2.f) / scale;
    if (a.pos_dim == 4) {
        kn[2] = (image ? a.scales1 : a.scales0)[src * n + r];
        kn[3] = (image ? a.oris1 : a.oris0)[src * n + r];
    }
    if (lane < 32) {
        float p = 0.f;
        for (int c = 0; c < a.pos_dim; ++c) p += kn[c] * a.Wr[lane * a.pos_dim + c];
        a.cosb[grow * 32 + lane] = cosf(p);
        a.sinb[grow * 32 + lane] = sinf(p);
    }
    if (lane == 0) a.ind[grow] = r;
    const float* d = (image ? a.desc1 : a.desc0) + (src * n + r) * a.input_dim;
    float* dst = (a.input_dim == 256) ? a.X + grow * 256 : a.Xin + grow * a.input_dim;
    for (int c = lane * 4; c < a.input_dim; c += 256) *reinterpret_cast<f32x4*>(dst + c) = *reinterpret_cast<const f32x4*>(d + c);
}

hipError_t launch_prep_bbox(const PrepArgs& a, hipStream_t s) {
    if (!a.size0 || !a.size1) hipLaunchKernelGGL(bbox_kernel, dim3(2 * a.rs.B), dim3(256), 0, s, a);
    return hipGetLastError();
}
hipError_t launch_prep(const PrepArgs& a, hipStream_t s) {
    if (a.input_dim % 4) return hipErrorInvalidValue;
    const int nseg = 2 * a.rs.B;
    if (!a.size0 || !a.size1) hipLaunchKernelGGL(bbox_kernel, dim3(nseg), dim3(256), 0, s, a);
    const int nmax = a.n0 > a.n1 ? a.n0 : a.n1;
    if (nmax > 0) hipLaunchKernelGGL(prep_kernel, dim3((nmax + 3) / 4, nseg), dim3(256), 0, s, a);
    return hipGetLastError();
}

__global__ __launch_bounds__(256) void ln_gelu_kernel(LnGeluArgs a) {
    const int wave = threadIdx.x >> 6, lane = threadIdx.x & 63;
    const int grow = blockIdx.x * 4 + wave;
    if (grow >= a.R) return;
    const TileLoc t = locate_tile(a.rs, grow, 1);
    if (t.r0 >= a.rs.len[t.seg]) return;
    if (a.rs.active && !a.rs.active[t.pair]) return;
    const float* h = a.h + (long long)grow * 512;
    f32x4 v0 = *reinterpret_cast<const f32x4*>(h + lane * 4);
    f32x4 v1 = *reinterpret_cast<const f32x4*>(h + 256 + lane * 4);
    float sum = v0[0] + v0[1] + v0[2] + v0[3] + v1[0] + v1[1] + v1[2] + v1[3];
    const float mean = wave_sum(sum) * (1.f / 512.f);
    v0 -= mean; v1 -= mean;
    float sq = v0[0] * v0[0] + v0[1] * v0[1] + v0[2] * v0[2] + v0[3] * v0[3] + v1[0] * v1[0] + v1[1] * v1[1] + v1[2] * v1[2] + v1[3] * v1[3];
    const float var = wave_sum(sq) * (1.f / 512.f);
    const float rstd = 1.f / sqrtf(var + 1e-5f);
    const f32x4 g0 = *reinterpret_cast<const f32x4*>(a.gamma + lane * 4), g1 = *reinterpret_cast<const f32x4*>(a.gamma + 256 + lane * 4);
    const f32x4 b0 = *reinterpret_cast<const f32x4*>(a.beta + lane * 4), b1 = *reinterpret_cast<const f32x4*>(a.beta + 256 + lane * 4);
    f32x4 y0, y1;
#pragma unroll
    for (int i = 0; i < 4; ++i) {
        const float u0 = v0[i] * rstd * g0[i] + b0[i], u1 = v1[i] * rstd * g1[i] + b1[i];
        y0[i] = 0.5f * u0 * (1.f + erff(u0 * 0.70710678118654752440f));
        y1[i] = 0.5f * u1 * (1.f + erff(u1 * 0.70710678118654752440f));
    }
    float* g = a.g + (long long)grow * 512;
    *reinterpret_cast<f32x4*>(g + lane * 4) = y0;
    *reinterpret_cast<f32x4*>(g + 256 + lane * 4) = y1;
}
hipError_t launch_ln_gelu(const LnGeluArgs& a, hipStream_t s) {
    hipLaunchKernelGGL(ln_gelu_kernel, dim3((a.R + 3) / 4), dim3(256), 0, s, a);
    return hipGetLastError();
}

__device__ __forceinline__ float act_apply(float z, int act) {
    if (act == 1) return 1.f / (1.f + expf(-z));
    if (act == 2) return fminf(z, 0.f) - log1pf(expf(-fabsf(z)));
    if (act == 3) return fminf(-z, 0.f) - log1pf(expf(-fabsf(z)));
    return z;
}
__global__ __launch_bounds__(256) void rowdot_kernel(RowDotArgs a, int R) {
    const int wave = threadIdx.x >> 6, lane = threadIdx.x & 63;
    const int grow = blockIdx.x * 4 + wave;
    if (grow >= R) return;
    const TileLoc t = locate_tile(a.rs, grow, 1);
    if (t.r0 >= a.rs.len[t.seg]) return;
    if (!a.ignore_active && a.rs.active && !a.rs.active[t.pair]) return;
    const int layer = a.layer_of_pair ? a.layer_of_pair[t.pair] : 0;
    const f32x4 x = *reinterpret_cast<const f32x4*>(a.X + (long long)grow * 256 + lane * 4);
    {
        const f32x4 w = *reinterpret_cast<const f32x4*>(a.w0 + (long long)layer * a.w_layer_stride + lane * 4);
        const float z = wave_sum(x[0] * w[0] + x[1] * w[1] + x[2] * w[2] + x[3] * w[3]) + a.b0[layer];
        if (lane == 0) a.out0[grow] = act_apply(z, a.act0);
    }
    if (a.w1) {
        const f32x4 w = *reinterpret_cast<const f32x4*>(a.w1 + (long long)layer * a.w_layer_stride + lane * 4);
        const float z = wave_sum(x[0] * w[0] + x[1] * w[1] + x[2] * w[2] + x[3] * w[3]) + a.b1[layer];
        if (lane == 0) a.out1[grow] = act_apply(z, a.act1);
    }
}
hipError_t launch_rowdot(const RowDotArgs& a, hipStream_t s) {
    const int R = a.rs.B * (a.rs.cap0 + a.rs.cap1);
    hipLaunchKernelGGL(rowdot_kernel, dim3((R + 3) / 4), dim3(256), 0, s, a, R);
    return hipGetLastError();
}

}
```

### lightglue_amd/csrc/lg_proj.hip

```cpp
#include "lg_proj_body.h"

namespace lg {

template <int PREC>
__device__ __forceinline__ void proj_load_tile(const float* X, const TileLoc& t, char* smA) {
    typedef typename PJ<PREC>::Tag Tag;
    constexpr int EPC = Tag::EPC;
    constexpr int KE = PJL<PREC>::KE, STAGES = PJL<PREC>::STAGES, TILE = PJL<PREC>::TILE, A_PLANE = PJL<PREC>::A_PLANE;
    constexpr int NV = EPC / 4;
    const int tid = threadIdx.x;
    const int srow = tid >> 3, sslot = tid & 7;
    const float* src = X + (long long)(t.grow0 + srow) * 256 + sslot * EPC;
    f32x4 hreg[STAGES][NV];
#pragma unroll
    for (int st = 0; st < STAGES; ++st)
#pragma unroll
        for (int j = 0; j < NV; ++j) hreg[st][j] = *reinterpret_cast<const f32x4*>(src + st * KE + 4 * j);
    const int off = pj_tile_off(srow, sslot);
#pragma unroll
    for (int st = 0; st < STAGES; ++st) {
        char* tile = smA + st * TILE;
        if constexpr (PREC == PREC_F32) {
            *reinterpret_cast<f32x4*>(tile + off) = hreg[st][0];
        } else if constexpr (PJ<PREC>::APART == 2) {
            u32x4 hi, lo;
            split8<Tag>(hreg[st][0], hreg[st][1], hi, lo);
            *reinterpret_cast<u32x4*>(tile + off) = hi;
            *reinterpret_cast<u32x4*>(tile + A_PLANE + off) = lo;
        } else {
            *reinterpret_cast<u32x4*>(tile + off) = pack8<Tag>(hreg[st][0], hreg[st][1]);
        }
    }
}

template <int PREC, class TA, int NTP, int NPASS>
__global__ __launch_bounds__(PTHREADS) void proj_kernel(ProjArgs a) {
    extern __shared__ __attribute__((aligned(16))) char smem[];
    char* smA = smem;

    const TileLoc t = locate_tile(a.rs, blockIdx.x, PBM);
    if (t.r0 >= a.rs.len[t.seg]) return;
    if (a.rs.active && !a.rs.active[t.pair]) return;
    const int tid = threadIdx.x, lane = tid & 63, w = __builtin_amdgcn_readfirstlane(tid >> 6);
    if (a.dbg && lane == 0) a.dbg[((long long)blockIdx.x * 8 + w) * 8] = clock64();
    RopeRows<4> rr;
    if constexpr (NTP == 3) proj_rope_load<4>(a, t, rr);
    proj_load_tile<PREC>(a.X, t, smA);
    proj_compute<PREC, TA, NTP, NPASS>(a, t, smA, 0, NTP == 3 ? &rr : nullptr);
}

template <int PREC, class TA>
__global__ __launch_bounds__(PTHREADS) void proj_first_kernel(ProjArgs a, PrepArgs pa) {
    typedef typename PJ<PREC>::Tag Tag;
    constexpr int EPC = Tag::EPC, NV = EPC / 4;
    constexpr int KE = PJL<PREC>::KE, STAGES = PJL<PREC>::STAGES, TILE = PJL<PREC>::TILE, A_PLANE = PJL<PREC>::A_PLANE, A_BYTES = PJL<PREC>::A_BYTES;
    extern __shared__ __attribute__((aligned(16))) char smem[];
    char* smA = smem;
    float* ldsC = reinterpret_cast<float*>(smem + A_BYTES);
    float* ldsS = ldsC + PBM * 32;

    const TileLoc t = locate_tile(a.rs, blockIdx.x, PBM);
    const int len = a.rs.len[t.seg];
    if (t.r0 >= len) return;
    if (a.rs.active && !a.rs.active[t.pair]) return;
    const int tid = threadIdx.x, lane = tid & 63, w = __builtin_amdgcn_readfirstlane(tid >> 6), lr = lane & 15, g = lane >> 4;
    const int image = t.seg & 1, n = image ? pa.n1 : pa.n0;
    const int srow = tid >> 3, sslot = tid & 7;
    const int r = t.r0 + srow, rc = r < len ? r : len - 1;
    const long long simg = source_image(pa.px, t.pair, image);
    const long long in_row = simg * n + rc;
    const float* src = (image ? pa.desc1 : pa.desc0) + in_row * 256 + sslot * EPC;
    f32x4 hreg[STAGES][NV];
#pragma unroll
    for (int st = 0; st < STAGES; ++st)
#pragma unroll
        for (int j = 0; j < NV; ++j) hreg[st][j] = *reinterpret_cast<const f32x4*>(src + st * KE + 4 * j);
    {
        const float* kp = (image ? pa.kpts1 : pa.kpts0) + in_row * 2;
        const float* szp = image ? pa.size1 : pa.size0;
        float sx, sy;
        if (szp) { sx = szp[simg * 2]; sy = szp[simg * 2 + 1]; }
        else { const float* bb = pa.bbox + t.seg * 4; sx = 1.f + bb[2] - bb[0]; sy = 1.f + bb[3] - bb[1]; }
        const float scale = fmaxf(sx, sy) / 2.f;
        float kn[4];
        kn[0] = (kp[0] - sx / 2.f) / scale;
        kn[1] = (kp[1] - sy / 2.f) / scale;
        if (pa.pos_dim == 4) {
            kn[2] = (image ? pa.scales1 : pa.scales0)[in_row];
            kn[3] = (image ? pa.oris1 : pa.oris0)[in_row];
        }
        f32x4 c4, s4;
#pragma unroll
        for (int f = 0; f < 4; ++f) {
            float p = 0.f;
            for (int c = 0; c < pa.pos_dim; ++c) p += kn[c] * pa.Wr[(sslot * 4 + f) * pa.pos_dim + c];
            c4[f] = cosf(p); s4[f] = sinf(p);
        }
        *reinterpret_cast<f32x4*>(ldsC + srow * 32 + sslot * 4) = c4;
        *reinterpret_cast<f32x4*>(ldsS + srow * 32 + sslot * 4) = s4;
        if (r < len) {
            const long long grow = t.grow0 + srow;
            *reinterpret_cast<f32x4*>(pa.cosb + grow * 32 + sslot * 4) = c4;
            *reinterpret_cast<f32x4*>(pa.sinb + grow * 32 + sslot * 4) = s4;
            if (sslot == 0) pa.ind[grow] = r;
        }
    }
    {
        const int off = pj_tile_off(srow, sslot);
        float* xdst = pa.X + (long long)(t.grow0 + srow) * 256 + sslot * EPC;
#pragma unroll
        for (int st = 0; st < STAGES; ++st) {
            char* tile = smA + st * TILE;
            if (r < len) {
#pragma unroll
                for (int j = 0; j < NV; ++j) *reinterpret_cast<f32x4*>(xdst + st * KE + 4 * j) = hreg[st][j];
            }
            if constexpr (PREC == PREC_F32) {
                *reinterpret_cast<f32x4*>(tile + off) = hreg[st][0];
            } else if constexpr (PJ<PREC>::APART == 2) {
                u32x4 hi, lo;
                split8<Tag>(hreg[st][0], hreg[st][1], hi, lo);
                *reinterpret_cast<u32x4*>(tile + off) = hi;
                *reinterpret_cast<u32x4*>(tile + A_PLANE + off) = lo;
            } else {
                *reinterpret_cast<u32x4*>(tile + off) = pack8<Tag>(hreg[st][0], hreg[st][1]);
            }
        }
    }
    __syncthreads();
    RopeRows<4> rr;
    {
        const int f0 = ((32 * w) & 63) / 2 + 4 * g;
#pragma unroll
        for (int mt = 0; mt < 4; ++mt) {
            const int row = pj_row<4>(mt, lr);
            rr.c[mt] = *reinterpret_cast<const f32x4*>(ldsC + row * 32 + f0);
            rr.s[mt] = *reinterpret_cast<const f32x4*>(ldsS + row * 32 + f0);
        }
    }
    proj_compute<PREC, TA, 3, 2>(a, t, smA, 0, &rr);
}
template <int PREC, class TA> static hipError_t launch_proj_first_t(const ProjArgs& a, const PrepArgs& pa, hipStream_t s) {
    const int R = a.rs.B * (a.rs.cap0 + a.rs.cap1);
    constexpr int smem = PJL<PREC>::A_BYTES + 2 * PBM * 32 * 4;
    auto kern = proj_first_kernel<PREC, TA>;
    hipError_t e = hipFuncSetAttribute(reinterpret_cast<const void*>(kern), hipFuncAttributeMaxDynamicSharedMemorySize, smem);
    if (e != hipSuccess) return e;
    hipLaunchKernelGGL(kern, dim3(R / PBM), dim3(PTHREADS), smem, s, a, pa);
    return hipGetLastError();
}
hipError_t launch_proj_first(int prec, int attn_prec, const ProjArgs& a, const PrepArgs& pa, hipStream_t s) {
    if (!(a.Nout == 768 && a.n_qk_groups == 2 && a.cosb && a.sinb) || pa.input_dim != 256) return hipErrorInvalidValue;
    if (prec == PREC_F32 && attn_prec == PREC_F32) return launch_proj_first_t<PREC_F32, float>(a, pa, s);
    if (prec == PREC_BF16 && attn_prec == PREC_BF16) return launch_proj_first_t<PREC_BF16, bf16_t>(a, pa, s);
    if (prec == PREC_F16 && attn_prec == PREC_F16) return launch_proj_first_t<PREC_F16, f16_t>(a, pa, s);
    if (prec == PREC_F16X3 && attn_prec == PREC_F16X3) return a.plane > 0 ? launch_proj_first_t<PREC_F16X3, f16_t>(a, pa, s) : hipErrorInvalidValue;
    if (prec == PREC_F16X3 && attn_prec == PREC_F16) return launch_proj_first_t<PREC_QKV_F16W2, f16_t>(a, pa, s);
    return hipErrorInvalidValue;
}

template <int PREC, class TA>
__global__ __launch_bounds__(PTHREADS) void proj_gather_kernel(ProjArgs a, GatherArgs ga) {
    typedef typename PJ<PREC>::Tag Tag;
    constexpr int EPC = Tag::EPC, NV = EPC / 4;
    constexpr int KE = PJL<PREC>::KE, STAGES = PJL<PREC>::STAGES, TILE = PJL<PREC>::TILE, A_PLANE = PJL<PREC>::A_PLANE, A_BYTES = PJL<PREC>::A_BYTES;
    extern __shared__ __attribute__((aligned(16))) char smem[];
    char* smA = smem;
    float* ldsC = reinterpret_cast<float*>(smem + A_BYTES);
    float* ldsS = ldsC + PBM * 32;

    const TileLoc t = locate_tile(a.rs, blockIdx.x, PBM);
    const int len = a.rs.len[t.seg];
    if (t.r0 >= len) return;
    if (a.rs.active && !a.rs.active[t.pair]) return;
    const int tid = threadIdx.x, lane = tid & 63, w = __builtin_amdgcn_readfirstlane(tid >> 6), lr = lane & 15, g = lane >> 4;
    const int srow = tid >> 3, sslot = tid & 7;
    const int r = t.r0 + srow, rc = r < len ? r : len - 1;
    const long long base = t.grow0 - t.r0;
    const int sr = ga.len_old[t.seg] >= 0 ? ga.src[base + rc] : rc;
    const long long in_row = base + sr;
    const float* src = ga.Xold + in_row * 256 + sslot * EPC;
    f32x4 hreg[STAGES][NV];
#pragma unroll
    for (int st = 0; st < STAGES; ++st)
#pragma unroll
        for (int j = 0; j < NV; ++j) hreg[st][j] = *reinterpret_cast<const f32x4*>(src + st * KE + 4 * j);
    {
        const f32x4 c4 = *reinterpret_cast<const f32x4*>(ga.cos_old + in_row * 32 + sslot * 4);
        const f32x4 s4 = *reinterpret_cast<const f32x4*>(ga.sin_old + in_row * 32 + sslot * 4);
        *reinterpret_cast<f32x4*>(ldsC + srow * 32 + sslot * 4) = c4;
        *reinterpret_cast<f32x4*>(ldsS + srow * 32 + sslot * 4) = s4;
        if (r < len) {
            const long long grow = t.grow0 + srow;
            *reinterpret_cast<f32x4*>(ga.cos_new + grow * 32 + sslot * 4) = c4;
            *reinterpret_cast<f32x4*>(ga.sin_new + grow * 32 + sslot * 4) = s4;
        }
    }
    {
        const int off = pj_tile_off(srow, sslot);
        float* xdst = ga.Xnew + (long long)(t.grow0 + srow) * 256 + sslot * EPC;
#pragma unroll
        for (int st = 0; st < STAGES; ++st) {
            char* tile = smA + st * TILE;
            if (r < len) {
#pragma unroll
                for (int j = 0; j < NV; ++j) *reinterpret_cast<f32x4*>(xdst + st * KE + 4 * j) = hreg[st][j];
            }
            if constexpr (PREC == PREC_F32) {
                *reinterpret_cast<f32x4*>(tile + off) = hreg[st][0];
            } else if constexpr (PJ<PREC>::APART == 2) {
                u32x4 hi, lo;
                split8<Tag>(hreg[st][0], hreg[st][1], hi, lo);
                *reinterpret_cast<u32x4*>(tile + off) = hi;
                *reinterpret_cast<u32x4*>(tile + A_PLANE + off) = lo;
            } else {
                *reinterpret_cast<u32x4*>(tile + off) = pack8<Tag>(hreg[st][0], hreg[st][1]);
            }
        }
    }
    __syncthreads();
    RopeRows<4> rr;
    {
        const int f0 = ((32 * w) & 63) / 2 + 4 * g;
#pragma unroll
        for (int mt = 0; mt < 4; ++mt) {
            const int row = pj_row<4>(mt, lr);
            rr.c[mt] = *reinterpret_cast<const f32x4*>(ldsC + row * 32 + f0);
            rr.s[mt] = *reinterpret_cast<const f32x4*>(ldsS + row * 32 + f0);
        }
    }
    proj_compute<PREC, TA, 3, 2>(a, t, smA, 0, &rr);
}
template <int PREC, class TA> static hipError_t launch_proj_gather_t(const ProjArgs& a, const GatherArgs& g, hipStream_t s) {
    const int R = a.rs.B * (a.rs.cap0 + a.rs.cap1);
    constexpr int smem = PJL<PREC>::A_BYTES + 2 * PBM * 32 * 4;
    auto kern = proj_gather_kernel<PREC, TA>;
    hipError_t e = hipFuncSetAttribute(reinterpret_cast<const void*>(kern), hipFuncAttributeMaxDynamicSharedMemorySize, smem);
    if (e != hipSuccess) return e;
    hipLaunchKernelGGL(kern, dim3(R / PBM), dim3(PTHREADS), smem, s, a, g);
    return hipGetLastError();
}
hipError_t launch_proj_gather(int prec, int attn_prec, const ProjArgs& a, const GatherArgs& g, hipStream_t s) {
    if (!(a.Nout == 768 && a.n_qk_groups == 2) || !g.Xold || !g.Xnew || !g.src || !g.len_old) return hipErrorInvalidValue;
    if (prec == PREC_F32 && attn_prec == PREC_F32) return launch_proj_gather_t<PREC_F32, float>(a, g, s);
    if (prec == PREC_BF16 && attn_prec == PREC_BF16) return launch_proj_gather_t<PREC_BF16, bf16_t>(a, g, s);
    if (prec == PREC_F16 && attn_prec == PREC_F16) return launch_proj_gather_t<PREC_F16, f16_t>(a, g, s);
    if (prec == PREC_F16X3 && attn_prec == PREC_F16X3) return a.plane > 0 ? launch_proj_gather_t<PREC_F16X3, f16_t>(a, g, s) : hipErrorInvalidValue;
    if (prec == PREC_F16X3 && attn_prec == PREC_F16) return launch_proj_gather_t<PREC_QKV_F16W2, f16_t>(a, g, s);
    return hipErrorInvalidValue;
}

template <int PREC>
__global__ __launch_bounds__(PTHREADS) void final_proj_kernel(FinalArgs a) {
    extern __shared__ __attribute__((aligned(16))) char smem[];
    const TileLoc t = locate_tile(a.rs, blockIdx.x, PBM);
    if (t.r0 >= a.rs.len[t.seg]) return;
    if (a.rs.active && !a.rs.active[t.pair]) return;
    proj_load_tile<PREC>((a.xsel && a.xsel[t.pair]) ? a.X2 : a.X, t, smem);
    final_compute<PREC>(a, t, smem);
}
template <int PREC> static hipError_t launch_final_t(const FinalArgs& a, hipStream_t s) {
    constexpr int smem = PJL<PREC>::A_BYTES;
    auto kern = final_proj_kernel<PREC>;
    hipError_t e = hipFuncSetAttribute(reinterpret_cast<const void*>(kern), hipFuncAttributeMaxDynamicSharedMemorySize, smem);
    if (e != hipSuccess) return e;
    hipLaunchKernelGGL(kern, dim3(a.R / PBM), dim3(PTHREADS), smem, s, a);
    return hipGetLastError();
}
hipError_t launch_final_proj(int prec, const FinalArgs& a, hipStream_t s) {
    switch (prec) {
        case PREC_F32: return launch_final_t<PREC_F32>(a, s);
        case PREC_BF16: return launch_final_t<PREC_BF16>(a, s);
        case PREC_F16: return launch_final_t<PREC_F16>(a, s);
        case PREC_F16X3: return launch_final_t<PREC_F16X3>(a, s);
    }
    return hipErrorInvalidValue;
}

template <int PREC, class TA, int NTP, int NPASS> static hipError_t launch_proj_t(const ProjArgs& a, hipStream_t s) {
    const int R = a.rs.B * (a.rs.cap0 + a.rs.cap1);
    constexpr int smem = PJL<PREC>::A_BYTES;
    auto kern = proj_kernel<PREC, TA, NTP, NPASS>;
    hipError_t e = hipFuncSetAttribute(reinterpret_cast<const void*>(kern), hipFuncAttributeMaxDynamicSharedMemorySize, smem);
    if (e != hipSuccess) return e;
    hipLaunchKernelGGL(kern, dim3(R / PBM), dim3(PTHREADS), smem, s, a);
    return hipGetLastError();
}
template <int PREC, class TA> static hipError_t launch_proj_n(const ProjArgs& a, hipStream_t s) {
    if (a.Nout == 768 && a.n_qk_groups == 2 && a.cosb && a.sinb) return launch_proj_t<PREC, TA, 3, 2>(a, s);
    if (a.Nout == 512 && a.n_qk_groups == 1) return launch_proj_t<PREC, TA, 2, 2>(a, s);
    return hipErrorInvalidValue;
}
hipError_t launch_proj(int prec, int attn_prec, const ProjArgs& a, hipStream_t s) {
    if (prec == PREC_F32 && attn_prec == PREC_F32) return launch_proj_n<PREC_F32, float>(a, s);
    if (prec == PREC_BF16 && attn_prec == PREC_BF16) return launch_proj_n<PREC_BF16, bf16_t>(a, s);
    if (prec == PREC_F16 && attn_prec == PREC_F16) return launch_proj_n<PREC_F16, f16_t>(a, s);
    if (prec == PREC_F16X3 && attn_prec == PREC_F16X3) return a.plane > 0 ? launch_proj_n<PREC_F16X3, f16_t>(a, s) : hipErrorInvalidValue;
    if (prec == PREC_F16X3 && attn_prec == PREC_F16) return launch_proj_n<PREC_QKV_F16W2, f16_t>(a, s);
    return hipErrorInvalidValue;
}

}
```

Measured before the change: 4258 image-pairs/s.

## Process pairs in chunks through all layers to keep activations cache-resident

Adds a pair-chunk plan that splits the batch into groups of pairs. Each group runs through every transformer layer before the next group starts, sized so that each group's per-layer working set (X, Q/K/V, scratch) fits a fixed last-level-cache budget. All row-space kernels gain a pair offset so they can address a sub-range of pairs. The aim is to cut HBM traffic from activations being evicted between layers. In exchange there are more kernel launches, smaller grids per launch, and weights are re-read once per chunk.

```diff
diff --git a/include/lightglue_amd.h b/include/lightglue_amd.h
--- a/include/lightglue_amd.h
+++ b/include/lightglue_amd.h
@@ -103,6 +103,8 @@
 
 int lg_engine_set_option(lg_engine* e, const char* key, int32_t value);
 
+int32_t lg_engine_pair_chunk(lg_engine* e, int32_t batch, int32_t n0, int32_t n1);
+
 int lg_debug_mfma_sustained(double* tflops, double* mhz, void* hip_stream);
 int lg_engine_debug_stop_after(lg_engine* e, int32_t step);
 int lg_engine_debug_read(lg_engine* e, const char* name, void* host_dst, int64_t max_bytes, int64_t* nbytes_out);
diff --git a/lightglue_amd/_cabi.py b/lightglue_amd/_cabi.py
--- a/lightglue_amd/_cabi.py
+++ b/lightglue_amd/_cabi.py
@@ -13,7 +13,7 @@
 
 EXPORTED_SYMBOLS = (
     "lg_last_error", "lg_version", "lg_engine_create", "lg_engine_destroy", "lg_engine_set_weight",
-    "lg_engine_finalize_weights", "lg_engine_reserve", "lg_engine_forward", "lg_unpack_wire", "lg_engine_set_option",
+    "lg_engine_finalize_weights", "lg_engine_reserve", "lg_engine_forward", "lg_unpack_wire", "lg_engine_set_option", "lg_engine_pair_chunk",
     "lg_engine_debug_stop_after", "lg_engine_debug_read", "lg_engine_debug_caps",
     "lg_profile_num_classes", "lg_profile_class_name", "lg_engine_profile_enable", "lg_engine_profile_read",
     "lg_sp_sample_descriptors", "lg_sp_detect_workspace_bytes", "lg_sp_detect",
@@ -112,6 +112,8 @@
     lib.lg_engine_forward.argtypes = [C.c_void_p, C.POINTER(LgForwardIO), C.c_void_p]
     lib.lg_unpack_wire.argtypes = [C.POINTER(LgUnpackIO), C.c_void_p]
     lib.lg_engine_set_option.argtypes = [C.c_void_p, C.c_char_p, C.c_int32]
+    lib.lg_engine_pair_chunk.argtypes = [C.c_void_p, C.c_int32, C.c_int32, C.c_int32]
+    lib.lg_engine_pair_chunk.restype = C.c_int32
     lib.lg_engine_debug_stop_after.argtypes = [C.c_void_p, C.c_int32]
     lib.lg_engine_debug_read.argtypes = [C.c_void_p, C.c_char_p, C.c_void_p, C.c_int64, C.POINTER(C.c_int64)]
     lib.lg_engine_debug_caps.argtypes = [C.c_void_p, C.POINTER(C.c_int32), C.POINTER(C.c_int32)]
diff --git a/lightglue_amd/csrc/lg_attention.hip b/lightglue_amd/csrc/lg_attention.hip
--- a/lightglue_amd/csrc/lg_attention.hip
+++ b/lightglue_amd/csrc/lg_attention.hip
@@ -48,8 +48,8 @@
         t = locate_tile(a.rs, v - w.head * ntile, ABM);
     } else {
         const int t0 = (a.rs.cap0 + ABM - 1) / ABM, t1 = (a.rs.cap1 + ABM - 1) / ABM, idx = v - w.head * ntile;
-        t.pair = idx / (t0 + t1);
-        const int rem = idx - t.pair * (t0 + t1);
+        const int lp = idx / (t0 + t1), rem = idx - lp * (t0 + t1);
+        t.pair = a.rs.pair0 + lp;
         t.image = rem >= t0 ? 1 : 0;
         t.r0 = (rem - t.image * t0) * ABM;
         t.seg = 2 * t.pair + t.image;
diff --git a/lightglue_amd/csrc/lg_common.h b/lightglue_amd/csrc/lg_common.h
--- a/lightglue_amd/csrc/lg_common.h
+++ b/lightglue_amd/csrc/lg_common.h
@@ -119,12 +119,13 @@
     int cap0, cap1;
     const int* len;
     const int* active;
+    int pair0 = 0;
 };
 struct TileLoc { int pair, image, seg, r0, grow0; };
 __device__ __forceinline__ TileLoc locate_tile(const RowSpace& rs, int tile, int tile_rows) {
     TileLoc t;
     const int per_pair = rs.cap0 + rs.cap1;
-    t.grow0 = tile * tile_rows;
+    t.grow0 = rs.pair0 * per_pair + tile * tile_rows;
     t.pair = t.grow0 / per_pair;
     const int rem = t.grow0 - t.pair * per_pair;
     t.image = rem >= rs.cap0 ? 1 : 0;
diff --git a/lightglue_amd/csrc/lg_debug.hip b/lightglue_amd/csrc/lg_debug.hip
--- a/lightglue_amd/csrc/lg_debug.hip
+++ b/lightglue_amd/csrc/lg_debug.hip
@@ -15,7 +15,7 @@
         HIPCHK(hipEventCreate(&sp.a)); HIPCHK(hipEventCreate(&sp.b));
         e->prof_pool.push_back(sp);
     }
-    e->prof_pool[e->prof_used].cls = cls;
+    e->prof_pool[e->prof_used].cls = cls; e->prof_pool[e->prof_used].counts = e->prof_counts;
     HIPCHK(hipEventRecord(e->prof_pool[e->prof_used].a, s));
     return LG_OK;
 }
@@ -37,7 +37,7 @@
         float ms = 0.f;
         HIPCHK(hipEventElapsedTime(&ms, e->prof_pool[i].a, e->prof_pool[i].b));
         e->prof_ms[e->prof_pool[i].cls] += ms;
-        e->prof_cnt[e->prof_pool[i].cls] += 1;
+        e->prof_cnt[e->prof_pool[i].cls] += e->prof_pool[i].counts ? 1 : 0;
     }
     e->prof_used = 0;
     return LG_OK;
diff --git a/lightglue_amd/csrc/lg_engine.h b/lightglue_amd/csrc/lg_engine.h
--- a/lightglue_amd/csrc/lg_engine.h
+++ b/lightglue_amd/csrc/lg_engine.h
@@ -62,6 +62,7 @@
     int tail_timing = 0; long long* TAILDBG = nullptr; long long* TAILDBG2 = nullptr;
     int* CFLAGS = nullptr; int compact_epoch = 0; bool cflags_clean = false;
     int tail_row_tiles = 0;
+    int pair_chunk = 0;
     bool attn_auto_rows = true;
     void* ws = nullptr; size_t ws_bytes = 0;
     int capB = 0, cap0 = 0, cap1 = 0;
@@ -79,7 +80,8 @@
     int debug_stop = -1;
     bool profiling = false, prof_open = false;
     int prof_only = -1;
-    struct ProfSpan { hipEvent_t a, b; int cls; };
+    struct ProfSpan { hipEvent_t a, b; int cls; bool counts; };
+    bool prof_counts = true;
     std::vector<ProfSpan> prof_pool;
     size_t prof_used = 0;
     double prof_ms[LG_PROF_NCLS] = {0};
diff --git a/lightglue_amd/csrc/lg_engine.hip b/lightglue_amd/csrc/lg_engine.hip
--- a/lightglue_amd/csrc/lg_engine.hip
+++ b/lightglue_amd/csrc/lg_engine.hip
@@ -119,6 +119,7 @@
     if (std::strcmp(key, "sim_chunk") == 0) { if (value < 0 || value % 64) return set_error(LG_ERR_INVALID, "sim_chunk: 0 or a multiple of 64"); e->sim_chunk = value; return LG_OK; }
     if (std::strcmp(key, "attn_rows") == 0) { if (value != 16 && value != 32 && value != 64) return set_error(LG_ERR_INVALID, "attn_rows must be 16, 32 or 64"); e->attn_rows = value; e->attn_auto_rows = false; return LG_OK; }
     if (std::strcmp(key, "tail_row_tiles") == 0) { if (value != 0 && value != 1 && value != 2 && value != 4) return set_error(LG_ERR_INVALID, "tail_row_tiles must be 0 (automatic), 1, 2 or 4"); e->tail_row_tiles = value; return LG_OK; }
+    if (std::strcmp(key, "pair_chunk") == 0) { if (value < 0) return set_error(LG_ERR_INVALID, "pair_chunk: 0 (automatic) or the pairs per chunk, >= 1"); e->pair_chunk = value; return LG_OK; }
     if (std::strcmp(key, "profile_only") == 0) { e->prof_only = value; return LG_OK; }
     if (std::strcmp(key, "tail_timing") == 0) { e->tail_timing = value; return LG_OK; }
     return set_error(LG_ERR_INVALID, std::string("unknown option '") + key + "'");
@@ -134,6 +135,22 @@
     }
     return best;
 }
+
+constexpr long long kPairChunkCacheBudget = 192LL << 20;
+constexpr long long kPairChunkMinRows = 2 * 256 * 64;
+long long layer_stack_row_bytes(const lg_engine* e) { return 2 * 256 * 4 + 3 * 256 * (long long)attn_elem_bytes(e->attn_prec) + 2 * 32 * 4; }
+int pair_chunk_plan(const lg_engine* e, bool eligible, int B, int c0, int c1) {
+    if (!eligible || B <= 1) return B;
+    if (e->pair_chunk > 0) return e->pair_chunk < B ? e->pair_chunk : B;
+    const long long rows = (long long)c0 + c1, per_pair = rows * layer_stack_row_bytes(e);
+    if (B * per_pair <= kPairChunkCacheBudget) return B;
+    for (int n = 2; n <= B; ++n) {
+        const int k = (B + n - 1) / n, last = B - (B - 1) / k * k;
+        if (k * per_pair <= kPairChunkCacheBudget && last * rows >= kPairChunkMinRows) return k;
+    }
+    return B;
+}
+bool chunk_eligible(const lg_engine* e, bool do_stop, bool do_prune) { return !do_stop && !do_prune && e->debug_stop < 0 && e->tail_timing == 0; }
 
 bool pruning_on(const lg_engine* e, const lg_forward_io* io) { return e->cfg.width_confidence > 0 && !(io->flags & LG_FLAG_NO_PRUNING); }
 bool indexed(const lg_forward_io* io) { return (io->flags & LG_FLAG_EXT) && (io->flags & LG_FLAG_INDEXED); }
@@ -194,6 +211,12 @@
 }
 }
 
+int32_t lg_engine_pair_chunk(lg_engine* e, int32_t batch, int32_t n0, int32_t n1) {
+    if (!e || batch < 1 || n0 < 0 || n1 < 0) { set_error(LG_ERR_INVALID, "bad argument"); return -1; }
+    const int c0 = round_up(n0 > 0 ? n0 : 1, 128), c1 = round_up(n1 > 0 ? n1 : 1, 128);
+    return pair_chunk_plan(e, chunk_eligible(e, e->cfg.depth_confidence > 0, e->cfg.width_confidence > 0), batch, c0, c1);
+}
+
 int lg_engine_forward(lg_engine* e, const lg_forward_io* io, void* hip_stream) {
     TRY(check_forward_io(e, io));
     hipStream_t s = static_cast<hipStream_t>(hip_stream);
@@ -207,6 +230,9 @@
     const int c0 = e->cur_cap0, c1 = e->cur_cap1, R = B * (c0 + c1);
     RowSpace rs_all{B, c0, c1, e->LEN, nullptr};
     RowSpace rs_act{B, c0, c1, e->LEN, e->ACTIVE};
+    const int chunk = pair_chunk_plan(e, chunk_eligible(e, do_stop, do_prune), B, c0, c1);
+    RowSpace rs_call = rs_all, rs_cact = rs_act;
+    int Rc = R;
     const int prec = e->cfg.precision, ap = e->attn_prec;
     int step = 0;
 #define STEP_DONE() do { if (e->debug_stop >= 0 && step >= e->debug_stop) return LG_OK; ++step; } while (0)
@@ -224,6 +250,7 @@
     p.Wr = e->Wr; p.pos_dim = 2 + 2 * (e->cfg.add_scale_ori ? 1 : 0);
     p.desc0 = io->desc0; p.desc1 = io->desc1; p.input_dim = e->cfg.input_dim;
     p.X = e->X; p.Xin = e->XIN; p.cosb = e->COS; p.sinb = e->SIN; p.ind = e->IND; p.bbox = e->BBOX;
+    e->prof_counts = true;
     TRY(prof_begin(e, PC_PREP, s));
     if (fuse_prep) HIPCHK(launch_prep_bbox(p, s)); else HIPCHK(launch_prep(p, s));
     auto gemm = [&](const RowSpace& rs, const float* A, int lda, const float* A2, int lda2, int K1, int K, const PackedW& W, size_t w_elems, const float* bias, int Nout, float* out) {
@@ -245,7 +272,7 @@
     bool gather_pending = false;
     auto make_proj = [&](int layer, int blk) {
         ProjArgs pj{};
-        pj.rs = rs_act; pj.X = Xs[xcur]; pj.R = R; pj.q = e->Q; pj.k = e->K; pj.vt = e->VT; pj.plane = qkv_plane;
+        pj.rs = rs_cact; pj.X = Xs[xcur]; pj.R = R; pj.q = e->Q; pj.k = e->K; pj.vt = e->VT; pj.plane = qkv_plane;
         const BlockWeights& bw = e->blocks[blk];
         pj.W = bw.qkv_p + (size_t)layer * bw.qkv_layer_bytes; pj.bias = bw.b_qkv + (size_t)layer * bw.Nout;
         pj.Nout = bw.Nout; pj.n_qk_groups = bw.n_qk_groups;
@@ -267,6 +294,9 @@
         f.layer_of_pair = per_pair ? e->FINAL_LAYER : nullptr; f.w_layer_bytes = (long long)e->final_layer_bytes;
         return f;
     };
+    for (int p0 = 0; p0 < B; p0 += chunk) {
+    rs_call.pair0 = rs_cact.pair0 = p0; rs_call.B = rs_cact.B = B - p0 < chunk ? B - p0 : chunk; Rc = rs_call.B * (c0 + c1);
+    e->prof_counts = p0 == 0;
     for (int i = 0; i < L; ++i) {
         for (int blk = 0; blk < 2; ++blk) {
             const BlockWeights& bw = e->blocks[blk];
@@ -275,11 +305,12 @@
                 pj.dbg = (e->tail_timing == 2 && blk == 0) ? e->TAILDBG : nullptr;
                 TRY(prof_begin(e, blk == 0 ? PC_GEMM_QKV_SELF : PC_GEMM_QKV_CROSS, s));
                 if (fuse_prep && i == 0 && blk == 0) {
-                    pj.rs = rs_all;
+                    pj.rs = rs_call;
                     if (launch_proj_first(prec, ap, pj, p, s) != hipSuccess) {
                         (void)hipGetLastError();
-                        HIPCHK(launch_prep(p, s));
-                        pj.rs = rs_act;
+                        PrepArgs pc = p; pc.rs = rs_call;
+                        HIPCHK(launch_prep(pc, s));
+                        pj.rs = rs_cact;
                         HIPCHK(launch_proj(prec, ap, pj, s));
                     }
                 }
@@ -297,15 +328,15 @@
             STEP_DONE();
             {
                 AttnArgs at{};
-                at.rs = rs_act; at.q = e->Q; at.k = e->K; at.vt = e->VT; at.plane = qkv_plane; at.ctx = e->CTX; at.R = R; at.cross = blk;
+                at.rs = rs_cact; at.q = e->Q; at.k = e->K; at.vt = e->VT; at.plane = qkv_plane; at.ctx = e->CTX; at.R = R; at.cross = blk;
                 at.dbg = (e->tail_timing == 3 && blk == 0) ? e->TAILDBG : nullptr;
-                at.rows_per_wave = (e->attn_auto_rows && R / 128 * 4 < 256) ? 16 : e->attn_rows; at.dma = e->attn_dma ? 1 : 0;
+                at.rows_per_wave = (e->attn_auto_rows && Rc / 128 * 4 < 256) ? 16 : e->attn_rows; at.dma = e->attn_dma ? 1 : 0;
                 PROFILED(blk == 0 ? PC_ATTN_SELF : PC_ATTN_CROSS, launch_attention(ap, at, s));
             }
             STEP_DONE();
             if (e->fused_tail) {
                 TailArgs ta{};
-                ta.rs = rs_act; ta.X = Xs[xcur]; ta.CTX = e->CTX; ta.range_flag = range_flag;
+                ta.rs = rs_cact; ta.X = Xs[xcur]; ta.CTX = e->CTX; ta.range_flag = range_flag;
                 ta.Wcat = bw.tail_cat + (size_t)i * e->tail_cat_layer_bytes; ta.bcat = bw.b_cat + (size_t)i * 512;
                 ta.gamma = bw.ln_g + (size_t)i * 512; ta.beta = bw.ln_b + (size_t)i * 512;
                 ta.W2 = bw.tail_2 + (size_t)i * e->tail_2_layer_bytes; ta.b2 = bw.b_f2 + (size_t)i * D;
@@ -322,13 +353,13 @@
                     }
                 }
                 ta.dbg = (e->tail_timing == 1 || (i == 0 && ((e->tail_timing == 5 && blk == 1) || (e->tail_timing == 6 && blk == 0)))) ? e->TAILDBG : nullptr;
-                ta.row_tiles = e->tail_row_tiles ? e->tail_row_tiles : tail_row_tiles_for(R);
+                ta.row_tiles = e->tail_row_tiles ? e->tail_row_tiles : tail_row_tiles_for(Rc);
                 if (fuse_next && (blk == 0 || (i + 1 < L && !prune_possible))) {
                     ta.next = make_proj(i + blk, blk ^ 1);
                     if (ta.dbg && e->tail_timing >= 5) ta.next.dbg = e->TAILDBG2;
                     proj_done = true;
                 } else if (fuse_next && blk == 1 && i + 1 == L && !do_stop) {
-                    ta.fin = make_final(rs_act, L - 1, false);
+                    ta.fin = make_final(rs_cact, L - 1, false);
                     final_done = true;
                 }
                 PROFILED(PC_TAIL, launch_tail(prec, ap, ta, s));
@@ -336,22 +367,22 @@
                 continue;
             }
             {
-                GemmArgs g = gemm(rs_act, e->CTX, D, nullptr, 0, D, D, bw.out, (size_t)i * D * D, bw.b_out + (size_t)i * D, D, e->MSG);
+                GemmArgs g = gemm(rs_cact, e->CTX, D, nullptr, 0, D, D, bw.out, (size_t)i * D * D, bw.b_out + (size_t)i * D, D, e->MSG);
                 PROFILED(PC_GEMM_OUT, launch_gemm(prec, EPI_STORE, g, s));
             }
             STEP_DONE();
             {
-                GemmArgs g = gemm(rs_act, e->X, D, e->MSG, D, D, 512, bw.f1, (size_t)i * 512 * 512, bw.b_f1 + (size_t)i * 512, 512, e->H1);
+                GemmArgs g = gemm(rs_cact, e->X, D, e->MSG, D, D, 512, bw.f1, (size_t)i * 512 * 512, bw.b_f1 + (size_t)i * 512, 512, e->H1);
                 PROFILED(PC_GEMM_FFN1, launch_gemm(prec, EPI_STORE, g, s));
             }
             STEP_DONE();
             {
-                LnGeluArgs ln{rs_act, e->H1, e->G, bw.ln_g + (size_t)i * 512, bw.ln_b + (size_t)i * 512, R};
+                LnGeluArgs ln{rs_cact, e->H1, e->G, bw.ln_g + (size_t)i * 512, bw.ln_b + (size_t)i * 512, R};
                 PROFILED(PC_LN_GELU, launch_ln_gelu(ln, s));
             }
             STEP_DONE();
             {
-                GemmArgs g = gemm(rs_act, e->G, 512, nullptr, 0, 512, 512, bw.f2, (size_t)i * D * 512, bw.b_f2 + (size_t)i * D, D, e->X);
+                GemmArgs g = gemm(rs_cact, e->G, 512, nullptr, 0, 512, 512, bw.f2, (size_t)i * D * 512, bw.b_f2 + (size_t)i * D, D, e->X);
                 PROFILED(PC_GEMM_FFN2, launch_gemm(prec, EPI_RESID, g, s));
             }
             STEP_DONE();
@@ -387,6 +418,8 @@
             PROFILED(PC_ADAPTIVE, launch_adapt(ad, s));
         }
     }
+    }
+    e->prof_counts = true;
     {
         if (!e->fused_tail) {
             RowDotArgs rd{};
diff --git a/lightglue_amd/csrc/lg_pointwise.hip b/lightglue_amd/csrc/lg_pointwise.hip
--- a/lightglue_amd/csrc/lg_pointwise.hip
+++ b/lightglue_amd/csrc/lg_pointwise.hip
@@ -3,7 +3,7 @@
 namespace lg {
 
 __global__ __launch_bounds__(256) void bbox_kernel(PrepArgs a) {
-    const int seg = blockIdx.x, image = seg & 1, pair = seg >> 1;
+    const int seg = 2 * a.rs.pair0 + blockIdx.x, image = seg & 1, pair = seg >> 1;
     const int n = image ? a.n1 : a.n0;
     const int live = a.rs.len[seg];
     const float* kp = (image ? a.kpts1 : a.kpts0) + (long long)source_image(a.px, pair, image) * n * 2;
@@ -26,7 +26,7 @@
 
 __global__ __launch_bounds__(256) void prep_kernel(PrepArgs a) {
     const int wave = threadIdx.x >> 6, lane = threadIdx.x & 63;
-    const int seg = blockIdx.y, image = seg & 1, pair = seg >> 1;
+    const int seg = 2 * a.rs.pair0 + blockIdx.y, image = seg & 1, pair = seg >> 1;
     const int n = image ? a.n1 : a.n0;
     const int r = blockIdx.x * 4 + wave;
     if (r >= a.rs.len[seg]) return;
@@ -72,11 +72,12 @@
 
 __global__ __launch_bounds__(256) void ln_gelu_kernel(LnGeluArgs a) {
     const int wave = threadIdx.x >> 6, lane = threadIdx.x & 63;
-    const int grow = blockIdx.x * 4 + wave;
-    if (grow >= a.R) return;
-    const TileLoc t = locate_tile(a.rs, grow, 1);
+    const int row = blockIdx.x * 4 + wave;
+    if (row >= a.rs.B * (a.rs.cap0 + a.rs.cap1)) return;
+    const TileLoc t = locate_tile(a.rs, row, 1);
     if (t.r0 >= a.rs.len[t.seg]) return;
     if (a.rs.active && !a.rs.active[t.pair]) return;
+    const int grow = t.grow0;
     const float* h = a.h + (long long)grow * 512;
     f32x4 v0 = *reinterpret_cast<const f32x4*>(h + lane * 4);
     f32x4 v1 = *reinterpret_cast<const f32x4*>(h + 256 + lane * 4);
@@ -100,7 +101,7 @@
     *reinterpret_cast<f32x4*>(g + 256 + lane * 4) = y1;
 }
 hipError_t launch_ln_gelu(const LnGeluArgs& a, hipStream_t s) {
-    hipLaunchKernelGGL(ln_gelu_kernel, dim3((a.R + 3) / 4), dim3(256), 0, s, a);
+    hipLaunchKernelGGL(ln_gelu_kernel, dim3((a.rs.B * (a.rs.cap0 + a.rs.cap1) + 3) / 4), dim3(256), 0, s, a);
     return hipGetLastError();
 }
 
@@ -112,9 +113,10 @@
 }
 __global__ __launch_bounds__(256) void rowdot_kernel(RowDotArgs a, int R) {
     const int wave = threadIdx.x >> 6, lane = threadIdx.x & 63;
-    const int grow = blockIdx.x * 4 + wave;
-    if (grow >= R) return;
-    const TileLoc t = locate_tile(a.rs, grow, 1);
+    const int row = blockIdx.x * 4 + wave;
+    if (row >= R) return;
+    const TileLoc t = locate_tile(a.rs, row, 1);
+    const int grow = t.grow0;
     if (t.r0 >= a.rs.len[t.seg]) return;
     if (!a.ignore_active && a.rs.active && !a.rs.active[t.pair]) return;
     const int layer = a.layer_of_pair ? a.layer_of_pair[t.pair] : 0;
diff --git a/lightglue_amd/csrc/lg_proj.hip b/lightglue_amd/csrc/lg_proj.hip
--- a/lightglue_amd/csrc/lg_proj.hip
+++ b/lightglue_amd/csrc/lg_proj.hip
@@ -264,7 +264,7 @@
     auto kern = final_proj_kernel<PREC>;
     hipError_t e = hipFuncSetAttribute(reinterpret_cast<const void*>(kern), hipFuncAttributeMaxDynamicSharedMemorySize, smem);
     if (e != hipSuccess) return e;
-    hipLaunchKernelGGL(kern, dim3(a.R / PBM), dim3(PTHREADS), smem, s, a);
+    hipLaunchKernelGGL(kern, dim3(a.rs.B * (a.rs.cap0 + a.rs.cap1) / PBM), dim3(PTHREADS), smem, s, a);
     return hipGetLastError();
 }
 hipError_t launch_final_proj(int prec, const FinalArgs& a, hipStream_t s) {
```

Measured after the change: 4149 image-pairs/s. 0.974x the previous value.
